# fluhus/frackyfrac

Hardware: NVIDIA B200
Metric: UniFrac sample-pairs/sec (unweighted) (higher is better)
Workload: dtype u8 x u8 -> s32 (tcgen05 kind::i8, exact), s64 chunk / row sums, f32 ratio / output

## Files before the change

frackyfrac_b200/csrc/embed.cu:

```cuda
#include "frc_internal.h"

namespace frc {

namespace {

constexpr int kThreads = 256;

__global__ void k_scatter_f64(const int64_t* __restrict__ row_ptr, const int32_t* __restrict__ col,
                              const double* __restrict__ val, int64_t s_base, int64_t s_end, double* E,
                              int64_t ld, int32_t* __restrict__ K, int32_t kp) {
  int64_t s = s_base + ((static_cast<int64_t>(blockIdx.x) * blockDim.x + threadIdx.x) >> 5);
  int lane = threadIdx.x & 31;
  if (s >= s_end) return;
  int64_t b = row_ptr[s], e = row_ptr[s + 1];
  for (int64_t k = b + lane; k < e; k += 32) {
    E[static_cast<int64_t>(col[k]) * ld + (s - s_base)] = val[k];
    if (K) K[((s >> 7) * kp + col[k]) * 128 + (s & 127)] = col[k];
  }
}

__global__ void k_level_sum_f64(const int32_t* __restrict__ nodes, const int32_t* __restrict__ child_ptr,
                                const int32_t* __restrict__ child_idx, double* E, int64_t ld,
                                int32_t* __restrict__ K, int32_t kp, int64_t s_base) {
  int32_t v = nodes[blockIdx.x];
  int64_t s = (static_cast<int64_t>(blockIdx.y) * blockDim.x + threadIdx.x) * 2;
  if (s >= ld) return;
  int32_t cb = child_ptr[v], ce = child_ptr[v + 1];
  double2 acc = make_double2(0.0, 0.0);
  for (int32_t c = cb; c < ce; ++c) {
    const double2 x = *reinterpret_cast<const double2*>(E + static_cast<int64_t>(child_idx[c]) * ld + s);
    acc.x = __dadd_rn(acc.x, x.x);
    acc.y = __dadd_rn(acc.y, x.y);
  }
  *reinterpret_cast<double2*>(E + static_cast<int64_t>(v) * ld + s) = acc;
  if (K) {
    const int64_t g = s_base + s;
    int32_t* const kt = K + (g >> 7) * kp * 128 + (g & 127);
    int2 key = make_int2(-1, -1);
    for (int32_t c = cb; c < ce; ++c) {
      const int2 x = *reinterpret_cast<const int2*>(kt + static_cast<int64_t>(child_idx[c]) * 128);
      key.x = max(key.x, x.x);
      key.y = max(key.y, x.y);
    }
    *reinterpret_cast<int2*>(kt + static_cast<int64_t>(v) * 128) = key;
  }
}

__global__ void k_totals_f64(const double* __restrict__ E, int32_t n_nodes, int64_t ld,
                             int64_t n_samples, double* __restrict__ total) {
  int64_t s = static_cast<int64_t>(blockIdx.x) * blockDim.x + threadIdx.x;
  if (s >= n_samples) return;
  double acc = 0.0;
  int32_t v = 0;
  for (; v + 8 <= n_nodes; v += 8) {
    double x[8];
#pragma unroll
    for (int u = 0; u < 8; ++u) x[u] = E[static_cast<int64_t>(v + u) * ld + s];
#pragma unroll
    for (int u = 0; u < 8; ++u) acc = __dadd_rn(acc, x[u]);
  }
  for (; v < n_nodes; ++v) acc = __dadd_rn(acc, E[static_cast<int64_t>(v) * ld + s]);
  total[s] = acc;
}

__global__ void k_normalize_f64(double* E, int32_t n_nodes, int64_t ld, int64_t n_samples,
                                const double* __restrict__ total) {
  int64_t s = static_cast<int64_t>(blockIdx.x) * blockDim.x + threadIdx.x;
  if (s >= n_samples) return;
  const double t = total[s];
  for (int32_t v = blockIdx.y; v < n_nodes; v += gridDim.y) {
    double x = E[static_cast<int64_t>(v) * ld + s];
    if (x != 0.0) E[static_cast<int64_t>(v) * ld + s] = __ddiv_rn(x, t);
  }
}

template <bool kMult>
__global__ void k_totals_partial_f64(const double* __restrict__ E, int32_t n_nodes, int64_t ld,
                                     const double* __restrict__ mult, double* __restrict__ partial) {
  int64_t s = static_cast<int64_t>(blockIdx.x) * blockDim.x + threadIdx.x;
  if (s >= ld) return;
  int32_t per = (n_nodes + gridDim.y - 1) / gridDim.y;
  int32_t v0 = blockIdx.y * per, v1 = min(n_nodes, v0 + per);
  auto term = [&](int32_t u) {
    const double x = E[static_cast<int64_t>(u) * ld + s];
    if constexpr (kMult) return mult[u] * x;
    else return x;
  };
  double a0 = 0.0, a1 = 0.0, a2 = 0.0, a3 = 0.0;
  int32_t v = v0;
  for (; v + 4 <= v1; v += 4) {
    a0 += term(v);
    a1 += term(v + 1);
    a2 += term(v + 2);
    a3 += term(v + 3);
  }
  for (; v < v1; ++v) a0 += term(v);
  partial[static_cast<int64_t>(blockIdx.y) * ld + s] = (a0 + a1) + (a2 + a3);
}

__global__ void k_weighted_operand(const double* __restrict__ E, const double* __restrict__ length,
                                   int32_t n_nodes, int64_t ld, const double* __restrict__ total,
                                   int prescale, float* __restrict__ A, double* __restrict__ partial) {
  int64_t s = static_cast<int64_t>(blockIdx.x) * blockDim.x + threadIdx.x;
  if (s >= ld) return;
  int32_t per = (n_nodes + gridDim.y - 1) / gridDim.y;
  int32_t v0 = blockIdx.y * per, v1 = min(n_nodes, v0 + per);
  const double t = total ? total[s] : 1.0;
  const double inv = t > 0.0 ? 1.0 / t : 0.0;
  double w = 0.0;
  for (int32_t v = v0; v < v1; ++v) {
    const double x = E[static_cast<int64_t>(v) * ld + s];
    const double a = total ? x * inv : x;
    const double la = length[v] * a;
    w += la;
    A[static_cast<int64_t>(v) * ld + s] = static_cast<float>(prescale ? la : a);
  }
  partial[static_cast<int64_t>(blockIdx.y) * ld + s] = w;
}

__global__ void k_weighted_operand_panels(const double* __restrict__ E, const double* __restrict__ length,
                                          int32_t n_nodes, int32_t kp, int64_t ld, int64_t s_base,
                                          const double* __restrict__ total, int prescale,
                                          float* __restrict__ Ap, double* __restrict__ partial) {
  int64_t ls = static_cast<int64_t>(blockIdx.x) * blockDim.x + threadIdx.x;
  if (ls >= ld) return;
  int32_t per = (n_nodes + gridDim.y - 1) / gridDim.y;
  int32_t v0 = blockIdx.y * per, v1 = min(n_nodes, v0 + per);
  const int64_t s = s_base + ls;
  float* dst = Ap + ((s >> 7) * kp) * 128 + (s & 127);
  const double t = total ? total[ls] : 1.0;
  const double inv = t > 0.0 ? 1.0 / t : 0.0;
  double w = 0.0;
  for (int32_t v = v0; v < v1; ++v) {
    const double x = E[static_cast<int64_t>(v) * ld + ls];
    const double a = total ? x * inv : x;
    const double la = length[v] * a;
    w += la;
    dst[static_cast<int64_t>(v) * 128] = static_cast<float>(prescale ? la : a);
  }
  if (blockIdx.y == gridDim.y - 1)
    for (int32_t v = n_nodes; v < kp; ++v) dst[static_cast<int64_t>(v) * 128] = 0.f;
  partial[static_cast<int64_t>(blockIdx.y) * ld + ls] = w;
}

__global__ void k_reduce_partials(const double* __restrict__ partial, int n_chunks, int64_t ld,
                                  int64_t n, double* __restrict__ out) {
  int64_t s = static_cast<int64_t>(blockIdx.x) * blockDim.x + threadIdx.x;
  if (s >= n) return;
  double acc = 0.0;
  for (int c = 0; c < n_chunks; ++c) acc += partial[static_cast<int64_t>(c) * ld + s];
  out[s] = acc;
}

// ... 142 lines not shown
#pragma unroll
    for (int u = 0; u < 8; ++u) {
      if (h + u < height) {
        if (n[u] >= 0) {
          const uint32_t x = colw[n[u]];
          if (x) atomicOr(colw + p[u], x);
        }
        __syncthreads();
      }
    }
  }
  uint32_t* dst = bitsT + static_cast<int64_t>(w) * kp;
  if (peers.n > 0) {
    const int64_t at = static_cast<int64_t>(w) * kp;
#pragma unroll 4
    for (int32_t k = tid; k < kp; k += 512) {
      const int32_t v = order[k];
      const uint32_t x = v >= 0 ? colw[v] : 0u;
#pragma unroll
      for (int pr = 0; pr < 8; ++pr)
        if (pr < peers.n) peers.p[pr][at + k] = x;
    }
  } else {
#pragma unroll 8
    for (int32_t k = tid; k < kp; k += 512) {
      const int32_t v = order[k];
      dst[k] = v >= 0 ? colw[v] : 0u;
    }
  }
  if (bitsS != nullptr) {
    const int32_t words = kp >> 5;
    for (int32_t g = warp; g * 128 < kp; g += 16) {
      uint32_t wout[4];
#pragma unroll
      for (int u = 0; u < 4; ++u) {
        const int32_t v = order[g * 128 + u * 32 + lane];
        const uint32_t wv = v >= 0 ? colw[v] : 0u;
        uint32_t mine = 0;
#pragma unroll
        for (int b = 0; b < 32; ++b) {
          const uint32_t bal = __ballot_sync(0xffffffffu, (wv >> b) & 1u);
          if (lane == b) mine = bal;
        }
        wout[u] = mine;
      }
      const int64_t srow = static_cast<int64_t>(w) * 32 + lane;
      *reinterpret_cast<uint4*>(bitsS + srow * words + g * 4) = make_uint4(wout[0], wout[1], wout[2], wout[3]);
    }
  }
}

__global__ void __launch_bounds__(32)
k_presence_rowsum_t(const uint32_t* __restrict__ bitsT, int32_t kp, int32_t per,
                    const double* __restrict__ lenq8, double* __restrict__ partial, int64_t ld, int32_t w0) {
  const int32_t w = blockIdx.x + w0, lane = threadIdx.x;
  const int32_t v0 = blockIdx.y * per, v1 = min(kp, v0 + per);
  const uint32_t* col = bitsT + static_cast<int64_t>(w) * kp;
  double a0 = 0.0, a1 = 0.0;
  for (int32_t v = v0; v < v1; v += 8) {
    const uint4 wa = *reinterpret_cast<const uint4*>(col + v), wb = *reinterpret_cast<const uint4*>(col + v + 4);
    const double2 l0 = *reinterpret_cast<const double2*>(lenq8 + v), l1 = *reinterpret_cast<const double2*>(lenq8 + v + 2);
    const double2 l2 = *reinterpret_cast<const double2*>(lenq8 + v + 4), l3 = *reinterpret_cast<const double2*>(lenq8 + v + 6);
    a0 += ((wa.x >> lane) & 1u) ? l0.x : 0.0;
    a1 += ((wa.y >> lane) & 1u) ? l0.y : 0.0;
    a0 += ((wa.z >> lane) & 1u) ? l1.x : 0.0;
    a1 += ((wa.w >> lane) & 1u) ? l1.y : 0.0;
    a0 += ((wb.x >> lane) & 1u) ? l2.x : 0.0;
    a1 += ((wb.y >> lane) & 1u) ? l2.y : 0.0;
    a0 += ((wb.z >> lane) & 1u) ? l3.x : 0.0;
    a1 += ((wb.w >> lane) & 1u) ? l3.y : 0.0;
  }
  partial[static_cast<int64_t>(blockIdx.y) * ld + w * 32 + lane] = a0 + a1;
}

__global__ void __launch_bounds__(32)
k_presence_rowsum_u8(const uint32_t* __restrict__ bitsT, int32_t kp, int32_t per,
                     const uint32_t* __restrict__ qam, const int32_t* __restrict__ col_exp,
                     double* __restrict__ partial, int64_t ld, int32_t w0, int32_t e_min,
                     long long* __restrict__ r_int) {
  const int32_t w = blockIdx.x + w0, lane = threadIdx.x;
  const int32_t v0 = blockIdx.y * per, v1 = min(kp, v0 + per);
  const uint32_t* col = bitsT + static_cast<int64_t>(w) * kp;
  const uint32_t m = 1u << lane;
  double tot = 0.0;
  unsigned long long tot_int = 0;
  for (int32_t blk = v0; blk < v1; blk += 128) {
    uint32_t a0 = 0, a1 = 0, a2 = 0, a3 = 0;
#pragma unroll 4
    for (int32_t v = blk; v < blk + 128; v += 8) {
      const uint4 wa = *reinterpret_cast<const uint4*>(col + v), wb = *reinterpret_cast<const uint4*>(col + v + 4);
      const uint4 qa = *reinterpret_cast<const uint4*>(qam + v), qb = *reinterpret_cast<const uint4*>(qam + v + 4);
      if (wa.x & m) a0 += qa.x;
      if (wa.y & m) a1 += qa.y;
      if (wa.z & m) a2 += qa.z;
      if (wa.w & m) a3 += qa.w;
      if (wb.x & m) a0 += qb.x;
      if (wb.y & m) a1 += qb.y;
      if (wb.z & m) a2 += qb.z;
      if (wb.w & m) a3 += qb.w;
    }
    const uint32_t sum = (a0 + a1) + (a2 + a3);
    const int32_t e = col_exp[blk];
    if (r_int) tot_int += static_cast<unsigned long long>(sum) << (e - e_min);
    else tot = fma(ldexp(1.0, e), static_cast<double>(sum), tot);
  }
  if (r_int) atomicAdd(reinterpret_cast<unsigned long long*>(r_int) + w * 32 + lane, tot_int);
  else partial[static_cast<int64_t>(blockIdx.y) * ld + w * 32 + lane] = tot;
}

__global__ void __launch_bounds__(256)
k_expand_operands_t(const uint32_t* __restrict__ bitsT, int32_t nw, int32_t kp,
                    int64_t np, const uint16_t* __restrict__ len_hi, const uint16_t* __restrict__ len_lo,
                    uint16_t* __restrict__ P, uint16_t* __restrict__ Bh, uint16_t* __restrict__ Bl,
                    const uint8_t* __restrict__ need) {
  __shared__ uint32_t words[8][64];
  const int32_t v0 = blockIdx.x * 64;
  const int32_t w0 = blockIdx.y * 8;
  const uint32_t nd = need ? need[blockIdx.y] : 3u;
  if (nd == 0u) return;
  for (int idx = threadIdx.x; idx < 512; idx += 256) {
    int word = idx >> 6, node = idx & 63;
    uint32_t x = 0;
    if (w0 + word < nw) x = bitsT[static_cast<int64_t>(w0 + word) * kp + v0 + node];
    words[word][node] = x;
  }
  __syncthreads();
  const int wi = threadIdx.x >> 5, lane = threadIdx.x & 31;
  const int32_t va = v0 + 2 * lane;
  const uint2 wab = *reinterpret_cast<const uint2*>(&words[wi][2 * lane]);
  const uint32_t wa = wab.x, wb = wab.y;
  const uint32_t hab = *reinterpret_cast<const uint32_t*>(len_hi + va);
  const uint32_t lab = *reinterpret_cast<const uint32_t*>(len_lo + va);
  const int64_t s0 = (static_cast<int64_t>(w0) + wi) * 32;
#pragma unroll 4
  for (int it = 0; it < 32; ++it) {
    const int64_t s = s0 + it;
    if (s >= np) break;
    const uint32_t m = (0xFFFFu & (0u - ((wa >> it) & 1u))) | (0xFFFF0000u & (0u - ((wb >> it) & 1u)));
    const int64_t o = s * kp + va;
    if (nd & 1u) *reinterpret_cast<uint32_t*>(P + o) = 0x3F803F80u & m;
    if (nd & 2u) {
      *reinterpret_cast<uint32_t*>(Bh + o) = hab & m;
      *reinterpret_cast<uint32_t*>(Bl + o) = lab & m;
    }
  }
}

__global__ void __launch_bounds__(256)
k_expand_operands_u8(const uint32_t* __restrict__ bitsT, int32_t nw, int32_t kp, int64_t np,
                     const uint8_t* __restrict__ qa, const uint8_t* __restrict__ qh,
                     const uint8_t* __restrict__ ql, uint8_t* __restrict__ A, uint8_t* __restrict__ Bh,
                     uint8_t* __restrict__ Bl, const uint8_t* __restrict__ need,
                     const uint32_t* __restrict__ qam, const int32_t* __restrict__ col_exp, int32_t e_min,
                     long long* __restrict__ r_int) {
  __shared__ __align__(16) uint32_t words[8][128];
  __shared__ __align__(16) uint32_t sq[128];
  const int32_t v0 = blockIdx.x * 128;
  const int32_t w0 = blockIdx.y * 8;
  const uint32_t nd = need ? need[blockIdx.y] : 3u;
  if (nd == 0u) return;
  for (int idx = threadIdx.x; idx < 1024; idx += 256) {
    int word = idx >> 7, node = idx & 127;
    uint32_t x = 0;
    if (w0 + word < nw) x = bitsT[static_cast<int64_t>(w0 + word) * kp + v0 + node];
    words[word][node] = x;
  }
  if (r_int != nullptr && threadIdx.x < 128) sq[threadIdx.x] = qam[v0 + threadIdx.x];
  __syncthreads();
  const int wi = threadIdx.x >> 5, lane = threadIdx.x & 31;
  const int32_t va = v0 + 4 * lane;
  const uint4 w4 = *reinterpret_cast<const uint4*>(&words[wi][4 * lane]);
  const uint32_t a4 = *reinterpret_cast<const uint32_t*>(qa + va);
  const uint32_t h4 = *reinterpret_cast<const uint32_t*>(qh + va);
  const uint32_t l4 = *reinterpret_cast<const uint32_t*>(ql + va);
  const int64_t s0 = (static_cast<int64_t>(w0) + wi) * 32;
#pragma unroll 4
  for (int it = 0; it < 32; ++it) {
    const int64_t s = s0 + it;
    if (s >= np) break;
    const uint32_t bits = ((w4.x >> it) & 1u) | (((w4.y >> it) & 1u) << 8) | (((w4.z >> it) & 1u) << 16) |
                          (((w4.w >> it) & 1u) << 24);
    const uint32_t m = bits * 0xFFu;
    const int64_t o = s * kp + va;
    if (nd & 1u) *reinterpret_cast<uint32_t*>(A + o) = a4 & m;
    if (nd & 2u) {
      *reinterpret_cast<uint32_t*>(Bh + o) = h4 & m;
      *reinterpret_cast<uint32_t*>(Bl + o) = l4 & m;
    }
  }
  if (r_int != nullptr) {
    const uint32_t m = 1u << lane;
    uint32_t a0 = 0, a1 = 0, a2 = 0, a3 = 0;
#pragma unroll 8
    for (int k = 0; k < 128; k += 4) {
      const uint4 w = *reinterpret_cast<const uint4*>(&words[wi][k]);
      const uint4 q = *reinterpret_cast<const uint4*>(&sq[k]);
      a0 += (w.x & m) ? q.x : 0u;
      a1 += (w.y & m) ? q.y : 0u;
      a2 += (w.z & m) ? q.z : 0u;
      a3 += (w.w & m) ? q.w : 0u;
    }
    const uint32_t sum = (a0 + a1) + (a2 + a3);
    const int64_t s = s0 + lane;
    if (sum != 0u && s < np)
      atomicAdd(reinterpret_cast<unsigned long long*>(r_int) + s,
                static_cast<unsigned long long>(sum) << (col_exp[v0] - e_min));
  }
}

__global__ void k_quantize_lengths(const double* __restrict__ len_col, const int32_t* __restrict__ col_exp,
                                   int32_t kp, uint8_t* __restrict__ qa, uint8_t* __restrict__ qh,
                                   uint8_t* __restrict__ ql, uint32_t* __restrict__ qam,
                                   double* __restrict__ lenq, double* __restrict__ qerr) {
  const int32_t k = blockIdx.x * blockDim.x + threadIdx.x;
  if (k >= kp) return;
  const double len = len_col[k];
  const int e = col_exp[k];
  const double x = ldexp(len, -e);
  int best_a = 0, best_m = 0;
  if (len > 0.0) {
    double best = 1e300;
    int a0 = static_cast<int>(ceil(x / 65535.0));
    if (a0 < 1) a0 = 1;
    for (int a = a0; a <= 255; ++a) {
      double m = rint(x / static_cast<double>(a));
      if (m > 65535.0) continue;
      if (m < 1.0) m = 1.0;
      const double err = fabs(static_cast<double>(a) * m - x);
      if (err < best) { best = err; best_a = a; best_m = static_cast<int>(m); }
    }
    if (best_a == 0) { best_a = 255; best_m = 65535; }
  }
  qa[k] = static_cast<uint8_t>(best_a);
  qh[k] = static_cast<uint8_t>(best_m >> 8);
  ql[k] = static_cast<uint8_t>(best_m & 255);
  qam[k] = static_cast<uint32_t>(best_a) * static_cast<uint32_t>(best_m);
  const double q = ldexp(static_cast<double>(best_a) * static_cast<double>(best_m), e);
  lenq[k] = q;
  const double err = fabs(q - len);
  qerr[k] = err > 2e-6 * len ? 1e6 * err : 0.0;
}

__global__ void __launch_bounds__(1024) k_sum_flag_u(const double* __restrict__ qerr, int32_t kp,
                                                     double* __restrict__ flag_u) {
  __shared__ double part[1024];
  double acc = 0.0;
  for (int32_t k = threadIdx.x; k < kp; k += 1024) acc += qerr[k];
  part[threadIdx.x] = acc;
  __syncthreads();
  for (int o = 512; o > 0; o >>= 1) {
    if (threadIdx.x < o) part[threadIdx.x] += part[threadIdx.x + o];
    __syncthreads();
  }
  if (threadIdx.x == 0) flag_u[0] = part[0];
}

}

int launch_embed_f64(const DevTree& t, const int32_t* level_ptr, const DevCsr& a, double* E,
                     int64_t ld, int64_t s_base, cudaStream_t s, int32_t* K, int32_t kp) {
  int launches = 0;
  cudaMemsetAsync(E, 0, sizeof(double) * ld * t.n_nodes, s);
  if (K) cudaMemsetAsync(K + (s_base >> 7) * kp * 128, 0xFF, sizeof(int32_t) * ld * kp, s);
  const int64_t s_end = s_base + ld < a.n_samples ? s_base + ld : a.n_samples;
  if (s_end > s_base && a.nnz > 0) {
    int64_t threads = (s_end - s_base) * 32;
    k_scatter_f64<<<static_cast<unsigned>((threads + kThreads - 1) / kThreads), kThreads, 0, s>>>(
        a.row_ptr, a.col, a.val, s_base, s_end, E, ld, K, kp);
    ++launches;
  }
  for (int32_t h = 1; h <= t.height; ++h) {
    int32_t b = level_ptr[h], e = level_ptr[h + 1];
    if (e == b) continue;
    dim3 grid(static_cast<unsigned>(e - b), static_cast<unsigned>((ld / 2 + kThreads - 1) / kThreads));
    k_level_sum_f64<<<grid, kThreads, 0, s>>>(t.level_nodes + b, t.child_ptr, t.child_idx, E, ld, K, kp, s_base);
    ++launches;
  }
  return launches;
}

static int pick_chunks(int32_t n_nodes) {
  int c = n_nodes / 256;
  return c < 1 ? 1 : (c > 64 ? 64 : c);
}

int launch_totals_fast_f64(const double* E, int32_t n_nodes, int64_t ld, const double* mult, double* total,
                           double* scratch, cudaStream_t s) {
  const int chunks = pick_chunks(n_nodes);
  dim3 grid(static_cast<unsigned>((ld + kThreads - 1) / kThreads), chunks);
  if (mult) k_totals_partial_f64<true><<<grid, kThreads, 0, s>>>(E, n_nodes, ld, mult, scratch);
  else k_totals_partial_f64<false><<<grid, kThreads, 0, s>>>(E, n_nodes, ld, nullptr, scratch);
  k_reduce_partials<<<static_cast<unsigned>((ld + kThreads - 1) / kThreads), kThreads, 0, s>>>(scratch, chunks, ld, ld,
                                                                                             total);
  return 2;
}

int launch_totals_f64(const double* E, int32_t n_nodes, int64_t ld, int64_t n_samples, double* total,
                      cudaStream_t s) {
  if (n_samples == 0) return 0;
  k_totals_f64<<<static_cast<unsigned>((n_samples + 127) / 128), 128, 0, s>>>(E, n_nodes, ld,
                                                                               n_samples, total);
  return 1;
}

int launch_normalize_f64(double* E, int32_t n_nodes, int64_t ld, int64_t n_samples,
                         const double* total, cudaStream_t s) {
  if (n_samples == 0) return 0;
  dim3 grid(static_cast<unsigned>((n_samples + kThreads - 1) / kThreads),
            static_cast<unsigned>(min(n_nodes, 512)));
  k_normalize_f64<<<grid, kThreads, 0, s>>>(E, n_nodes, ld, n_samples, total);
  return 1;
}


int launch_weighted_operand(const double* E, const double* length, int32_t n_nodes, int32_t kp,
                            int64_t ld, int64_t n_samples, const double* total, bool prescale,
                            float* A, double* W, double* scratch, cudaStream_t s) {
  int chunks = pick_chunks(n_nodes);
  if (kp > n_nodes)
    cudaMemsetAsync(A + static_cast<int64_t>(n_nodes) * ld, 0, sizeof(float) * ld * (kp - n_nodes), s);
  dim3 grid(static_cast<unsigned>((ld + kThreads - 1) / kThreads), chunks);
  k_weighted_operand<<<grid, kThreads, 0, s>>>(E, length, n_nodes, ld, total, prescale ? 1 : 0, A,
                                               scratch);
  k_reduce_partials<<<static_cast<unsigned>((ld + kThreads - 1) / kThreads), kThreads, 0, s>>>(
      scratch, chunks, ld, ld, W);
  (void)n_samples;
  return 2;
}
int launch_weighted_operand_panels(const double* E, const double* length, int32_t n_nodes, int32_t kp,
                                   int64_t ld, int64_t s_base, const double* total, bool prescale, float* Ap,
                                   double* W, double* scratch, cudaStream_t s) {
  int chunks = pick_chunks(n_nodes);
  dim3 grid(static_cast<unsigned>((ld + kThreads - 1) / kThreads), chunks);
  k_weighted_operand_panels<<<grid, kThreads, 0, s>>>(E, length, n_nodes, kp, ld, s_base, total, prescale ? 1 : 0,
                                                      Ap, scratch);
  k_reduce_partials<<<static_cast<unsigned>((ld + kThreads - 1) / kThreads), kThreads, 0, s>>>(
      scratch, chunks, ld, ld, W + s_base);
  return 2;
}
int weighted_scratch_chunks(int32_t n_nodes) { return pick_chunks(n_nodes); }

int launch_embed_bits(const DevTree& t, const int32_t* level_ptr, const DevCsr& a, uint32_t* bits,
                      int32_t nw, cudaStream_t s) {
  int launches = 0;
  cudaMemsetAsync(bits, 0, sizeof(uint32_t) * static_cast<int64_t>(nw) * t.n_nodes, s);
  if (a.n_samples > 0 && a.nnz > 0) {
    int64_t threads = a.n_samples * 32;
    k_scatter_bits<<<static_cast<unsigned>((threads + kThreads - 1) / kThreads), kThreads, 0, s>>>(
        a.row_ptr, a.col, a.n_samples, bits, nw);
    ++launches;
  }
  for (int32_t h = 1; h <= t.height; ++h) {
    int32_t b = level_ptr[h], e = level_ptr[h + 1];
    if (e == b) continue;
    dim3 grid(static_cast<unsigned>(e - b), static_cast<unsigned>((nw + 127) / 128));
    k_level_or<<<grid, 128, 0, s>>>(t.level_nodes + b, t.child_ptr, t.child_idx, bits, nw);
    ++launches;
  }
  return launches;
}

int launch_presence_rowsum(const uint32_t* bits, int32_t n_nodes, int32_t nw, const double* lenq,
                           double* r, double* scratch, cudaStream_t s) {
  int chunks = pick_chunks(n_nodes);
  dim3 grid(nw, chunks);
  k_presence_rowsum<<<grid, 32, 0, s>>>(bits, n_nodes, nw, lenq, scratch);
  int64_t ld = static_cast<int64_t>(nw) * 32;
  k_reduce_partials<<<static_cast<unsigned>((ld + kThreads - 1) / kThreads), kThreads, 0, s>>>(
      scratch, chunks, ld, ld, r);
  return 2;
}

int launch_expand_operands(const uint32_t* bits, int32_t n_nodes, int32_t nw, int32_t kp, int64_t np,
                           const uint16_t* len_hi, const uint16_t* len_lo, uint16_t* P, uint16_t* Bh,
                           uint16_t* Bl, cudaStream_t s) {
  dim3 grid(kp / 64, static_cast<unsigned>((np + 255) / 256));
  k_expand_operands<<<grid, 256, 0, s>>>(bits, n_nodes, nw, kp, np, len_hi, len_lo, P, Bh, Bl);
  return 1;
}


void embed_setup() {
  cudaFuncSetAttribute(k_embed_presence_fused<true>, cudaFuncAttributeMaxDynamicSharedMemorySize, 200 * 1024);
}

int64_t presence_node_scratch_words(int32_t n_nodes, int32_t nw) {
  return static_cast<size_t>(n_nodes) * 4 <= 200 * 1024 ? 0 : static_cast<int64_t>(n_nodes) * nw;
}

int launch_embed_presence_fused(const DevTree& t, const int32_t* level_ptr_dev, const DevCsr& a,
                                int32_t nw, int32_t w0, int32_t w_count, int32_t kp, const int32_t* order,
                                uint32_t* node_scratch, uint32_t* bitsT, uint32_t* bitsS, const PeerPtrs& peers,
                                cudaStream_t s) {
  (void)nw;
  const size_t smem = (static_cast<size_t>(t.n_nodes) * 4 + 15) & ~size_t(15);
  if (smem <= 200 * 1024) {
    k_embed_presence_fused<true><<<w_count, 512, smem, s>>>(a.row_ptr, a.col, a.n_samples, t.level_nodes,
                                                            t.level_parent, level_ptr_dev, t.height, t.n_nodes, kp,
                                                            order, node_scratch, bitsT, w0, bitsS, peers);
  } else {
    k_embed_presence_fused<false><<<w_count, 512, 0, s>>>(a.row_ptr, a.col, a.n_samples, t.level_nodes,
                                                          t.level_parent, level_ptr_dev, t.height, t.n_nodes, kp,
                                                          order, node_scratch, bitsT, w0, bitsS, peers);
  }
  return 1;
}

int launch_presence_rowsum_t(const uint32_t* bitsT, int32_t n_nodes, int32_t nw, int32_t w0, int32_t w_count,
                             int32_t kp, const double* lenq, const uint32_t* qam, const int32_t* col_exp,
                             double* partial, double* r, int32_t e_min, long long* r_int, cudaStream_t s) {
  const int64_t np = static_cast<int64_t>(nw) * 32;
  const int chunks = pick_chunks(n_nodes);
  dim3 g(w_count, chunks);
  const int64_t s0 = static_cast<int64_t>(w0) * 32, ns = static_cast<int64_t>(w_count) * 32;
  if (qam) {
    const int32_t per = static_cast<int32_t>(round_up((kp + chunks - 1) / chunks, 128));
    if (r_int) cudaMemsetAsync(r_int + s0, 0, sizeof(long long) * ns, s);
    k_presence_rowsum_u8<<<g, 32, 0, s>>>(bitsT, kp, per, qam, col_exp, partial, np, w0, e_min, r_int);
    if (r_int) return 1;
  } else {
    const int32_t per = static_cast<int32_t>(round_up((kp + chunks - 1) / chunks, 8));
    k_presence_rowsum_t<<<g, 32, 0, s>>>(bitsT, kp, per, lenq, partial, np, w0);
  }
  k_reduce_partials<<<static_cast<unsigned>((ns + kThreads - 1) / kThreads), kThreads, 0, s>>>(partial + s0, chunks, np,
                                                                                              ns, r + s0);
  return 2;
}

int launch_expand_operands_t(const uint32_t* bitsT, int32_t nw, int32_t kp, int64_t np, bool i8,
                             const void* q0, const void* q1, const void* q2, void* P, void* Bh, void* Bl,
                             const uint8_t* need, const uint32_t* qam, const int32_t* col_exp, int32_t e_min,
                             long long* r_int, cudaStream_t s) {
  if (i8) {
    if (r_int) cudaMemsetAsync(r_int, 0, sizeof(long long) * np, s);
    dim3 grid(kp / 128, static_cast<unsigned>((np + 255) / 256));
    k_expand_operands_u8<<<grid, 256, 0, s>>>(bitsT, nw, kp, np, static_cast<const uint8_t*>(q0),
                                              static_cast<const uint8_t*>(q1), static_cast<const uint8_t*>(q2),
                                              static_cast<uint8_t*>(P), static_cast<uint8_t*>(Bh),
                                              static_cast<uint8_t*>(Bl), need, qam, col_exp, e_min, r_int);
  } else {
    (void)q0;
    dim3 grid(kp / 64, static_cast<unsigned>((np + 255) / 256));
    k_expand_operands_t<<<grid, 256, 0, s>>>(bitsT, nw, kp, np, static_cast<const uint16_t*>(q1),
                                             static_cast<const uint16_t*>(q2), static_cast<uint16_t*>(P),
                                             static_cast<uint16_t*>(Bh), static_cast<uint16_t*>(Bl), need);
  }
  return 1;
}

int launch_quantize_lengths(const double* len_col, const int32_t* col_exp, int32_t kp, uint8_t* qa,
                            uint8_t* qh, uint8_t* ql, uint32_t* qam, double* lenq, double* qerr, double* flag_u,
                            cudaStream_t s) {
  k_quantize_lengths<<<(kp + 127) / 128, 128, 0, s>>>(len_col, col_exp, kp, qa, qh, ql, qam, lenq, qerr);
  k_sum_flag_u<<<1, 1024, 0, s>>>(qerr, kp, flag_u);
  return 2;
}

}
```

frackyfrac_b200/csrc/frc_internal.h:

```cpp
#pragma once
#include <cuda_runtime.h>
#include <cstdint>
#include <string>

namespace frc {

constexpr int kTile = 128;
constexpr int kKBlock = 64;

inline int64_t round_up(int64_t x, int64_t m) { return (x + m - 1) / m * m; }
inline int64_t tri(int64_t i) { return i * (i - 1) / 2; }

struct DevTree {
  int32_t n_nodes = 0;
  int32_t height = 0;
  const int32_t* parent = nullptr;
  const double* length = nullptr;
  const int32_t* child_ptr = nullptr;
  const int32_t* child_idx = nullptr;
  const int32_t* level_nodes = nullptr;
  const int32_t* level_parent = nullptr;
};

struct DevCsr {
  int64_t n_samples = 0;
  int64_t nnz = 0;
  const int64_t* row_ptr = nullptr;
  const int32_t* col = nullptr;
  const double* val = nullptr;
};

struct PeerPtrs {
  uint32_t* p[8] = {nullptr, nullptr, nullptr, nullptr, nullptr, nullptr, nullptr, nullptr};
  int n = 0;
  int self = 0;
};

struct Tile { int32_t ti, tj; };

struct Exceptions {
  unsigned long long* count = nullptr;
  int64_t* index = nullptr;
  double* value = nullptr;
  int32_t cap = 0;
};

int launch_embed_f64(const DevTree& t, const int32_t* level_ptr_host, const DevCsr& a, double* E,
                     int64_t ld, int64_t s_base, cudaStream_t s, int32_t* K = nullptr, int32_t kp = 0);
int launch_totals_f64(const double* E, int32_t n_nodes, int64_t ld, int64_t n_samples,
                      double* total, cudaStream_t s);
int launch_totals_fast_f64(const double* E, int32_t n_nodes, int64_t ld, const double* mult, double* total,
                           double* scratch, cudaStream_t s);
int launch_normalize_f64(double* E, int32_t n_nodes, int64_t ld, int64_t n_samples,
                         const double* total, cudaStream_t s);
int launch_weighted_operand(const double* E, const double* length, int32_t n_nodes, int32_t kp,
                            int64_t ld, int64_t n_samples, const double* total, bool prescale,
                            float* A, double* W, double* scratch, cudaStream_t s);
int launch_weighted_operand_panels(const double* E, const double* length, int32_t n_nodes, int32_t kp,
                                   int64_t ld, int64_t s_base, const double* total, bool prescale, float* Ap,
                                   double* W, double* scratch, cudaStream_t s);
int weighted_scratch_chunks(int32_t n_nodes);

int launch_embed_bits(const DevTree& t, const int32_t* level_ptr_host, const DevCsr& a,
                      uint32_t* bits, int32_t nw, cudaStream_t s);
int launch_presence_rowsum(const uint32_t* bits, int32_t n_nodes, int32_t nw, const double* lenq,
                           double* r, double* scratch, cudaStream_t s);
int launch_expand_operands(const uint32_t* bits, int32_t n_nodes, int32_t nw, int32_t kp,
                           int64_t np, const uint16_t* len_hi, const uint16_t* len_lo,
                           uint16_t* P, uint16_t* Bh, uint16_t* Bl, cudaStream_t s);

int64_t presence_node_scratch_words(int32_t n_nodes, int32_t nw);
void embed_setup();
int launch_embed_presence_fused(const DevTree& t, const int32_t* level_ptr_dev, const DevCsr& a,
                                int32_t nw, int32_t w0, int32_t w_count, int32_t kp, const int32_t* order,
                                uint32_t* node_scratch, uint32_t* bitsT, uint32_t* bitsS, const PeerPtrs& peers,
                                cudaStream_t s);
int launch_presence_rowsum_t(const uint32_t* bitsT, int32_t n_nodes, int32_t nw, int32_t w0, int32_t w_count,
                             int32_t kp, const double* lenq, const uint32_t* qam, const int32_t* col_exp,
                             double* partial, double* r, int32_t e_min, long long* r_int, cudaStream_t s);
int launch_expand_operands_t(const uint32_t* bitsT, int32_t nw, int32_t kp, int64_t np, bool i8,
                             const void* q0, const void* q1, const void* q2, void* P, void* Bh, void* Bl,
                             const uint8_t* need, const uint32_t* qam, const int32_t* col_exp, int32_t e_min,
                             long long* r_int, cudaStream_t s);
int launch_quantize_lengths(const double* len_col, const int32_t* col_exp, int32_t kp, uint8_t* qa,
                            uint8_t* qh, uint8_t* ql, uint32_t* qam, double* lenq, double* qerr, double* flag_u,
                            cudaStream_t s);

struct Comm;
bool comm_unique_id(char* id128, std::string* err);
Comm* comm_create(const char* id128, int rank, int world, std::string* err);
void comm_destroy(Comm* c);
int comm_rank(const Comm* c);
int comm_world(const Comm* c);
bool comm_all_gather_inplace(Comm* c, void* const* bufs, const size_t* bytes_per_rank, int n, cudaStream_t s,
                             std::string* err);

bool comm_all_gather_host(Comm* c, const void* mine, size_t bytes, void* all, cudaStream_t s, std::string* err);
bool comm_barrier(Comm* c, cudaStream_t s, std::string* err);

int launch_exact_pairs(const double* E, const double* length, int32_t n_nodes, int64_t ld,
                       bool weighted, int64_t first, int64_t count, double* out, cudaStream_t s);
int launch_postorder_lists(const double* E, const int32_t* post_order, int32_t n_nodes, int64_t ld, int64_t n_samples,
                           int64_t* list_ptr, int32_t* list_id, double* list_val, cudaStream_t s);
int launch_unsorted_pairs(const int64_t* list_ptr, const int32_t* list_id, const double* list_val,
                          const double* length, int64_t first, int64_t count, double* out, cudaStream_t s);

void widen_band(const float* src, double* dst, int64_t n, bool stream_stores);

struct PanelMap {
  const float* shard[16] = {nullptr, nullptr, nullptr, nullptr, nullptr, nullptr, nullptr, nullptr,
                            nullptr, nullptr, nullptr, nullptr, nullptr, nullptr, nullptr, nullptr};
  int32_t n_shards = 0;
  int32_t tiles_per_shard = 0;
};
int launch_weighted_tiles(const PanelMap& A, int64_t ld, int32_t kp, const float* lenf, bool prescaled,
                          const double* W, const Tile* tiles, int32_t n_tiles, int64_t n_samples,
                          int64_t first, float* out, double flag_below, uint32_t* flagged,
                          unsigned long long* n_flagged, int num_sms, cudaStream_t s, const int32_t* K = nullptr);
int launch_weighted_fixup(const DevCsr& a, const DevTree& t, const double* total, const double* W,
                          const uint32_t* flagged, const unsigned long long* n_flagged,
                          unsigned long long* count_host, int64_t first, long long* ws, int ws_ctas, float* out,
                          const Exceptions& ex, cudaStream_t s, const int32_t* K = nullptr, int32_t kp = 0);
void weighted_setup();

struct TcOperands;
struct TcChunks {
  const int32_t* end = nullptr;
  const double* scale = nullptr;
  const int32_t* shift = nullptr;
  int32_t n = 0;
  bool biased = false;
};
TcOperands* tc_operands_create(const void* P, const void* Bh, const void* Bl, int64_t np, int32_t kp,
                               bool i8, const TcChunks& chunks, const double* len_col, const double* flag_u,
                               std::string* err);
TcOperands* tc_operands_create_bits(const uint32_t* bitsS, int64_t np, int32_t kp, const uint8_t* qa,
                                    const uint8_t* qh, const uint8_t* ql, const TcChunks& chunks,
                                    const double* len_col, const double* flag_u, const long long* r_int,
                                    double unit, std::string* err);
void tc_operands_set_int(TcOperands* o, const long long* r_int, double unit);
void tc_operands_destroy(TcOperands* o);
int tc_chunk_kblocks();
int launch_unweighted_tc(const TcOperands* ops, const double* r, const Tile* tiles, int32_t n_tiles,
                         int64_t n_samples, int64_t first, float* out, double flag_below,
                         uint32_t* flagged, unsigned long long* n_flagged, int num_sms, cudaStream_t s);
int launch_unweighted_fixup(const TcOperands* ops, const uint32_t* flagged,
                            const unsigned long long* n_flagged, unsigned long long* count_host,
                            int64_t first, float* out, const Exceptions& ex, int num_sms, cudaStream_t s);
bool tc_setup(std::string* err);

}
```

frackyfrac_b200/csrc/job.cu:

```cuda
#include <algorithm>
#include <atomic>
#include <chrono>
#include <climits>
#include <cmath>
#include <cstdio>
#include <cstdlib>
#include <cstring>
#include <functional>
#include <memory>
#include <string>
#include <thread>
#include <vector>

#if defined(__x86_64__)
#include <immintrin.h>
#endif

#include "../../include/frcfrc_cuda.h"
#include "frc_internal.h"
#include "host_pool.h"
#include "plan.h"

using namespace frc;
using frc_host::Pool;
// ... 66 lines not shown
  int ws_slab = 0;
  bool uw_bf16 = false;
  bool u8_acc_f64 = false;
  bool feed_bits = false;
  bool embed_levels = false;
  int peer_push = -1;
  int group_binades = 3;
  int shard = -1;
  int capacity = -1;
  static Knobs read() {
    Knobs k;
    auto num = [](const char* name, int dflt) { const char* e = getenv(name); return e && *e ? atoi(e) : dflt; };
    auto is = [](const char* name, const char* v) { const char* e = getenv(name); return e && !strcmp(e, v); };
    k.trace = getenv("FRC_TRACE") != nullptr;
    k.bands_per_rank = std::max(0, num("FRC_BANDS", 0));
    k.widen_threads = std::max(0, num("FRC_WIDEN_THREADS", 0));
    k.ws_slab = std::max(0, num("FRC_WS_SLAB", 0));
    k.uw_bf16 = is("FRC_UW_KERNEL", "bf16");
    k.u8_acc_f64 = is("FRC_U8_ACC", "f64");
    k.feed_bits = is("FRC_UW_FEED", "bits");
    k.embed_levels = num("FRC_EMBED_LEVELS", 0) == 1;
    k.peer_push = num("FRC_PEER_PUSH", -1);
    k.group_binades = num("FRC_U8_GROUP_BINADES", 3);
    k.shard = num("FRC_SHARD", -1);
    k.capacity = num("FRC_CAPACITY", -1);
    return k;
  }
};

struct DeviceGuard {
  int prev = -1;
  DeviceGuard() { if (cudaGetDevice(&prev) != cudaSuccess) { prev = -1; cudaGetLastError(); } }
  ~DeviceGuard() { if (prev >= 0) cudaSetDevice(prev); }
};

}

struct DevCtx {
  int device = 0;
  int num_sms = 0;
  cudaStream_t stream[4] = {nullptr, nullptr, nullptr, nullptr};
  Arena dev, pin, sym;
};

struct frc_ctx {
  std::vector<DevCtx*> devs;
  Arena pin;
  std::unique_ptr<Pool> pool;
  std::vector<std::vector<int64_t>> stamps;
  int64_t stamp_epoch = 0;
  bool in_use = false;
  bool peer_ok = false;
  Comm* comm = nullptr;
  std::vector<std::vector<char*>> sym_peer;
};

namespace {

struct Slot {
  double* dev64 = nullptr;
  double* host64 = nullptr;
  float* dev32 = nullptr;
  float* host32 = nullptr;
  uint32_t* flagged = nullptr;
  unsigned long long* n_flagged_host = nullptr;
  Exceptions ex;
  cudaEvent_t k0 = nullptr, k1 = nullptr, k2 = nullptr, done = nullptr;
  int band = -1;
};

struct Seg { size_t off = 0, bytes = 0; };
struct SegAlloc {
  size_t total = 0;
  Seg operator()(size_t bytes) { Seg s{total, bytes}; total += (bytes + 255) & ~size_t(255); return s; }
};

struct Shared {
  frc_opts_t opts{};
  Knobs knobs;
  int64_t N = 0, np = 0, nnz = 0;
  int32_t B = 0, kp = 0, nw = 0;
  bool exact = false, weighted = false, prescale = true, need_val = false;
  bool unsorted_l = false;
  bool keyed = false;
  bool node_mult = false;
  bool d2h = true;
  int n_parts = 1;
  int world = 1, rank0 = 0;
  enum Exchange { kNone, kInProcess, kNccl } exchange = kNone;
  bool fused_embed = true, bits_feed = false;
  bool capacity = false;
  ShardPlan shards;
  ColumnPlan cols;
  std::vector<Band> bands;
  std::vector<int32_t> level_ptr;
  int32_t tree_height = 0;
  char* stage_in = nullptr;
  Seg in_rowptr, in_parent, in_len, in_cptr, in_cidx, in_lvl, in_lpar, in_lptr, in_lenf, in_post, in_mult, in_col, in_val;
  size_t in_bytes = 0;
  char* stage_plan = nullptr;
  Seg pl_q0, pl_hi, pl_lo, pl_lenq, pl_order, pl_cexp, pl_lcol, pl_cend, pl_cscale, pl_cshift;
  size_t plan_bytes = 0;
};

}

struct frc_job;

namespace {

struct Part {
  frc_job* job = nullptr;
  const Shared* sh = nullptr;
  DevCtx* dc = nullptr;
  int index = 0;
  int owner = 0;
  int rc = FRC_OK;
  std::string err;
  frc_info_t info{};

  std::vector<int> mine;
  std::vector<Band> bands;
  std::vector<Tile> tiles;

  int32_t shard_w0 = 0, shard_nw = 0;
  int64_t csr_k0 = 0, csr_k1 = 0;
  PanelMap pm;
  struct CapGroup {
    int shard = 0;
    int64_t first = 0, count = 0;
    int32_t tile_off = 0;
    std::vector<int32_t> coff;
    float* out = nullptr;
    uint32_t* flagged = nullptr;
    unsigned long long* cnt = nullptr;
    unsigned long long* n_flagged_host = nullptr;
    Exceptions ex;
    cudaEvent_t done = nullptr;
    bool counted = false;
  };
  std::vector<CapGroup> cap;
  std::vector<int> band_group;
  float* d_V[2] = {nullptr, nullptr};
  std::vector<cudaEvent_t> ev_fetch, ev_used;

  DevTree dtree;
  DevCsr dcsr;
  char* d_in = nullptr;
  char* d_plan = nullptr;
  Tile* d_tiles = nullptr;
  int32_t* d_level_ptr = nullptr;
  int32_t* d_post = nullptr;
  unsigned long long* d_flag_counts = nullptr;
  int64_t ws_slab = 0;
  bool peer_push = false;
  uint32_t* d_bits2[2] = {nullptr, nullptr};
  PeerPtrs peers[2];
  int64_t run_count = 0;
  void *d_q0 = nullptr, *d_q1 = nullptr, *d_q2 = nullptr;
  int32_t *d_order = nullptr, *d_col_exp = nullptr;
  uint32_t* d_qam = nullptr;
  uint32_t* d_bitsS = nullptr;
  long long* d_r_int = nullptr;
  long long* d_fix_ws[2] = {nullptr, nullptr};
  uint8_t* d_need = nullptr;
  double *d_lenq = nullptr, *d_len_col = nullptr, *d_flag_u = nullptr, *d_qerr = nullptr;
  TcChunks d_chunks;
  float* d_lenf = nullptr;
  const double* d_mult = nullptr;
  double *d_E = nullptr, *d_total = nullptr, *d_W = nullptr, *d_r = nullptr, *d_scratch = nullptr;
  float* d_A = nullptr;
  int32_t* d_K = nullptr;
  uint32_t *d_bits = nullptr, *d_node_scratch = nullptr;
  void *d_P = nullptr, *d_Bh = nullptr, *d_Bl = nullptr;
  TcOperands* tc = nullptr;
  int64_t* d_list_ptr = nullptr;
  int32_t* d_list_id = nullptr;
  double* d_list_val = nullptr;
  int64_t list_cap = 0;

  Slot slots[kSlots];
  int n_slots = 0;
  int64_t max_band = 1;
  size_t next_enqueue = 0, next_deliver = 0;
  cudaEvent_t ev_h2d0 = nullptr, ev_h2d1 = nullptr, ev_embed0 = nullptr, ev_embed1 = nullptr;
  cudaEvent_t ev_run1 = nullptr, ev_join = nullptr, ev_bits = nullptr, ev_rsum = nullptr;
  cudaEvent_t ev_shard = nullptr;
  bool run_timed = false, embed_timed = false;
  std::chrono::steady_clock::time_point t_host0;
};

}

struct frc_job {
  frc_ctx* ctx = nullptr;
  bool own_ctx = false;
  Shared sh;
  std::vector<std::unique_ptr<Part>> parts;
  std::string err;
  frc_info_t info{};
  struct Item { int part, idx; };
  std::vector<Item> order;
  size_t next_item = 0;
  int held_part = -1;
  int held_slot = -1;
  int64_t held_first = 0, held_count = 0;
  std::vector<int64_t> ex_index;
  std::vector<double> ex_value;
  int read_mode = 0;
  double* wide = nullptr;
  int64_t piece_first = 0, piece_off = 0, piece_end = 0;
  double create_ms = 0;
};

namespace {

#define PART_CUDA(p, expr)                                                                   \
  do {                                                                                       \
    cudaError_t _e = (expr);                                                                 \
    if (_e != cudaSuccess) {                                                                 \
      (p)->err = std::string(#expr) + ": " + cudaGetErrorString(_e);                         \
      cudaGetLastError();                                                                    \
      return (p)->rc = (_e == cudaErrorMemoryAllocation ? FRC_ERR_OOM : FRC_ERR_CUDA);       \
    }                                                                                        \
  } while (0)

int pfail(Part* p, int code, const std::string& msg) { p->err = msg; return p->rc = code; }
int fail(frc_job* j, int code, const std::string& msg) { j->err = msg; return code; }

template <class T>
T* dev_alloc(Part* p, size_t n) {
  cudaError_t e = cudaSuccess;
  void* q = p->dc->dev.alloc(n * sizeof(T), &e);
  if (!q) {
    p->err = "device allocation of " + std::to_string(n * sizeof(T)) + " bytes failed: " + cudaGetErrorString(e);
    p->rc = FRC_ERR_OOM;
  }
  return static_cast<T*>(q);
}
template <class T>
T* pin_alloc(Part* p, size_t n) {
  cudaError_t e = cudaSuccess;
  void* q = p->dc->pin.alloc(n * sizeof(T), &e);
  if (!q) {
    p->err = "pinned host allocation of " + std::to_string(n * sizeof(T)) + " bytes failed: " + cudaGetErrorString(e);
    p->rc = FRC_ERR_OOM;
  }
  return static_cast<T*>(q);
}

int for_parts(frc_job* j, const std::function<int(Part*)>& fn) {
  const int n = static_cast<int>(j->parts.size());
  if (n == 1) {
    cudaSetDevice(j->parts[0]->dc->device);
    fn(j->parts[0].get());
  } else {
    Pool* pool = j->ctx->pool.get();
    const int T = std::min(n, pool->size());
    std::atomic<int> next{0};
    pool->run(T, [&](int) {
      for (int k = next.fetch_add(1); k < n; k = next.fetch_add(1)) {
        cudaSetDevice(j->parts[k]->dc->device);
        fn(j->parts[k].get());
      }
    });
  }
  for (auto& p : j->parts)
    if (p->rc) { j->err = p->err; return p->rc; }
  return FRC_OK;
}

int sym_sync(Part* p, bool* usable) {
  frc_ctx* c = p->job->ctx;
  DevCtx* dc = p->dc;
  const int world = comm_world(c->comm), rank = comm_rank(c->comm);
  char failed = 0;
  while (c->sym_peer.size() < dc->sym.blocks.size()) {
    const size_t b = c->sym_peer.size();
    cudaIpcMemHandle_t mine;
    memset(&mine, 0, sizeof(mine));
    if (cudaIpcGetMemHandle(&mine, dc->sym.blocks[b].p) != cudaSuccess) { cudaGetLastError(); failed = 1; }
    std::vector<cudaIpcMemHandle_t> all(world);
    std::string cerr;
    if (!comm_all_gather_host(c->comm, &mine, sizeof(mine), all.data(), dc->stream[0], &cerr))
      return pfail(p, FRC_ERR_CUDA, cerr);
    std::vector<char*> bases(world, nullptr);
    for (int r = 0; r < world; ++r) {
      if (r == rank) { bases[r] = dc->sym.blocks[b].p; continue; }
      void* q = nullptr;
      if (failed || cudaIpcOpenMemHandle(&q, all[r], cudaIpcMemLazyEnablePeerAccess) != cudaSuccess) {
        cudaGetLastError();
        failed = 1;
        q = nullptr;
      }
      bases[r] = static_cast<char*>(q);
    }
    c->sym_peer.push_back(bases);
  }
  for (auto& blk : c->sym_peer)
    for (char* base : blk)
      if (!base) failed = 1;
  std::vector<char> flags(world, 0);
  std::string cerr;
  if (!comm_all_gather_host(c->comm, &failed, 1, flags.data(), dc->stream[0], &cerr)) return pfail(p, FRC_ERR_CUDA, cerr);
  *usable = true;
  for (char f : flags) if (f) *usable = false;
  return FRC_OK;
}

struct ShardArray {
  void* (*on)(const Part*);
  size_t sample_bytes;
  bool copy = true;
};
template <auto M> void* part_array(const Part* q) { return q->*M; }

int exchange_shard(Part* p, const std::vector<ShardArray>& arrs, const Range& rg, cudaStream_t s) {
  const Shared& sh = *p->sh;
  if (sh.exchange == Shared::kNone) return FRC_OK;
  const size_t n = static_cast<size_t>(rg.s1 - rg.s0);
  const int others = (sh.exchange == Shared::kNccl ? sh.world : sh.n_parts) - 1;
  std::vector<void*> bufs;
  std::vector<size_t> bytes;
  for (const ShardArray& a : arrs) {
    p->info.gather_bytes += static_cast<int64_t>(n * a.sample_bytes) * others;
    if (a.copy) { bufs.push_back(a.on(p)); bytes.push_back(n * a.sample_bytes); }
  }
  if (sh.exchange == Shared::kNccl) {
    Comm* comm = p->job->ctx->comm;
    std::string cerr;
    const bool ok = bufs.empty() ? comm_barrier(comm, s, &cerr)
                                 : comm_all_gather_inplace(comm, bufs.data(), bytes.data(), static_cast<int>(bufs.size()), s, &cerr);
    return ok ? FRC_OK : pfail(p, FRC_ERR_CUDA, cerr);
  }
  for (int q = 0; q < sh.n_parts; ++q) {
    if (q == p->index) continue;
    const Part* o = p->job->parts[q].get();
    for (const ShardArray& a : arrs) {
      if (!a.copy) continue;
      const size_t off = rg.s0 * a.sample_bytes;
      PART_CUDA(p, cudaMemcpyPeerAsync(static_cast<char*>(a.on(o)) + off, o->dc->device, static_cast<char*>(a.on(p)) + off,
                                       p->dc->device, n * a.sample_bytes, s));
    }
  }
  return FRC_OK;
}

int embed_stage1(Part* p) {
  const Shared& sh = *p->sh;
  DevCtx* dc = p->dc;
  frc_ctx* c = p->job->ctx;
  cudaStream_t s = dc->stream[0];
  int launches = 0;
  p->t_host0 = std::chrono::steady_clock::now();
  if (p->d_flag_counts)
    PART_CUDA(p, cudaMemsetAsync(p->d_flag_counts, 0, sizeof(unsigned long long) * (p->mine.size() + 1), s));
  PART_CUDA(p, cudaEventRecord(p->ev_embed0, s));
  p->info.gather_bytes = 0;
  const bool inproc = sh.exchange == Shared::kInProcess;
  if (sh.exact) {
    launches += launch_embed_f64(p->dtree, sh.level_ptr.data(), p->dcsr, p->d_E, sh.np, 0, s);
    if (sh.opts.normalize == 1 && sh.weighted) {
      launches += launch_totals_f64(p->d_E, sh.B, sh.np, sh.N, p->d_total, s);
      launches += launch_normalize_f64(p->d_E, sh.B, sh.np, sh.N, p->d_total, s);
    }
    if (sh.unsorted_l) {
      launches += launch_postorder_lists(p->d_E, p->d_post, sh.B, sh.np, sh.N, p->d_list_ptr, nullptr, nullptr, s);
      int64_t total = 0;
      PART_CUDA(p, cudaMemcpyAsync(&total, p->d_list_ptr + sh.N, sizeof(int64_t), cudaMemcpyDeviceToHost, s));
      PART_CUDA(p, cudaStreamSynchronize(s));
      if (total > p->list_cap) {
        p->list_cap = total;
        if (!(p->d_list_id = dev_alloc<int32_t>(p, static_cast<size_t>(total) + 1))) return p->rc;
        if (!(p->d_list_val = dev_alloc<double>(p, static_cast<size_t>(total) + 1))) return p->rc;
      }
      launches += launch_postorder_lists(p->d_E, p->d_post, sh.B, sh.np, sh.N, p->d_list_ptr, p->d_list_id,
                                         p->d_list_val, s);
    }
    p->info.embed_bytes = 2LL * sh.B * sh.np * 8 + 12LL * sh.nnz;
  } else if (sh.weighted) {
    const bool norm = sh.opts.normalize == 1;
    std::vector<ShardArray> arrs;
    if (!sh.capacity) arrs.push_back({part_array<&Part::d_A>, sizeof(float) * sh.kp});
    arrs.push_back({part_array<&Part::d_W>, sizeof(double)});
    if (norm) arrs.push_back({part_array<&Part::d_total>, sizeof(double)});
    if (sh.keyed) arrs.push_back({part_array<&Part::d_K>, sizeof(int32_t) * sh.kp});
    int64_t built = 0;
    for (const Range& rg : sh.shards.ranges[p->owner]) {
      built += rg.s1 - rg.s0;
      const int64_t shift = (rg.slot * sh.shards.shard_rows - rg.s0) * sh.kp;
      float* Ap = p->d_A + shift;
      int32_t* Kp = sh.keyed ? p->d_K + shift : nullptr;
      for (int64_t sb = rg.s0; sb < rg.s1; sb += p->ws_slab) {
        const int64_t ld = std::min<int64_t>(p->ws_slab, rg.s1 - sb);
        launches += launch_embed_f64(p->dtree, sh.level_ptr.data(), p->dcsr, p->d_E, ld, sb, s, Kp, sh.kp);
        if (norm) launches += launch_totals_fast_f64(p->d_E, sh.B, ld, p->d_mult, p->d_total + sb, p->d_scratch, s);
        launches += launch_weighted_operand_panels(p->d_E, p->dtree.length, sh.B, sh.kp, ld, sb,
                                                   norm ? p->d_total + sb : nullptr, sh.prescale, Ap, p->d_W,
                                                   p->d_scratch, s);
      }
      if (exchange_shard(p, arrs, rg, s)) return p->rc;
    }
    p->pm = PanelMap{};
    if (sh.capacity) {
      p->pm.n_shards = sh.shards.n_shards;
      p->pm.tiles_per_shard = static_cast<int32_t>(sh.shards.shard_rows / kTile);
      for (int k = 0; k < sh.shards.n_shards; ++k)
        if (sh.shards.owner[k] == p->owner) p->pm.shard[k] = p->d_A + sh.shards.slot[k] * sh.shards.shard_rows * sh.kp;
    } else {
      p->pm.shard[0] = p->d_A;
    }
    p->info.embed_bytes = 2LL * sh.B * built * (sh.keyed ? 12 : 8) + 12LL * (p->csr_k1 - p->csr_k0);
  } else if (sh.fused_embed) {
    const int cur = static_cast<int>(p->run_count & 1);
    if (p->peer_push) {
      p->d_bits = p->d_bits2[cur];
      if (p->run_count == 0) {
        std::string cerr;
        if (!comm_barrier(c->comm, s, &cerr)) return pfail(p, FRC_ERR_CUDA, cerr);
      }
    }
    ++p->run_count;
    PeerPtrs peers;
    if (p->peer_push) peers = p->peers[cur];
    else if (inproc && !sh.bits_feed) {
      peers.n = sh.n_parts; peers.self = p->index;
      for (int q = 0; q < sh.n_parts; ++q) peers.p[q] = p->job->parts[q]->d_bits;
    }
    launches += launch_embed_presence_fused(p->dtree, p->d_level_ptr, p->dcsr, sh.nw, p->shard_w0, p->shard_nw,
                                            sh.kp, p->d_order, p->d_node_scratch, p->d_bits, p->d_bitsS, peers, s);
    const bool rowsum_in_expand = sh.cols.intacc && !sh.bits_feed;
    const bool split = sh.exchange == Shared::kNone && !rowsum_in_expand;
    cudaStream_t rs = split ? dc->stream[1] : s;
    if (split) {
      PART_CUDA(p, cudaEventRecord(p->ev_bits, s));
      PART_CUDA(p, cudaStreamWaitEvent(rs, p->ev_bits, 0));
    }
    if (!rowsum_in_expand)
      launches += launch_presence_rowsum_t(p->d_bits, sh.B, sh.nw, p->shard_w0, p->shard_nw, sh.kp, p->d_lenq,
                                           sh.cols.i8 ? p->d_qam : nullptr, p->d_col_exp, p->d_scratch, p->d_r,
                                           sh.cols.e_min, sh.cols.intacc ? p->d_r_int : nullptr, rs);
    std::vector<ShardArray> arrs;
    if (!rowsum_in_expand)
      arrs.push_back({sh.cols.intacc ? part_array<&Part::d_r_int> : part_array<&Part::d_r>, sizeof(double)});
    arrs.push_back({sh.bits_feed ? part_array<&Part::d_bitsS> : part_array<&Part::d_bits>, sizeof(uint32_t) * sh.kp / 32,
                    peers.n == 0});
    if (exchange_shard(p, arrs, sh.shards.ranges[p->owner][0], s)) return p->rc;
    if (sh.exchange != Shared::kNone) {
      p->info.embed_bytes = 2LL * sh.B * p->shard_nw * 4 + 4LL * (p->csr_k1 - p->csr_k0);
    }
  }
  PART_CUDA(p, cudaGetLastError());
  if (inproc) PART_CUDA(p, cudaEventRecord(p->ev_shard, s));
  p->info.kernel_launches += launches;
  return FRC_OK;
}

int embed_stage2(Part* p) {
  const Shared& sh = *p->sh;
  DevCtx* dc = p->dc;
  cudaStream_t s = dc->stream[0];
  int launches = 0;
  if (sh.exchange == Shared::kInProcess)
    for (auto& o : p->job->parts)
      if (o.get() != p) PART_CUDA(p, cudaStreamWaitEvent(s, o->ev_shard, 0));
  if (!sh.exact && !sh.weighted) {
    if (sh.fused_embed) {
      const bool rowsum_in_expand = sh.cols.intacc && !sh.bits_feed;
      if (!sh.bits_feed)
        launches += launch_expand_operands_t(p->d_bits, sh.nw, sh.kp, sh.np, sh.cols.i8, p->d_q0, p->d_q1, p->d_q2,
                                             p->d_P, p->d_Bh, p->d_Bl, p->d_need, p->d_qam, p->d_col_exp, sh.cols.e_min,
                                             rowsum_in_expand ? p->d_r_int : nullptr, s);
      if (sh.exchange == Shared::kNone) {
        if (!rowsum_in_expand) {
          PART_CUDA(p, cudaEventRecord(p->ev_rsum, dc->stream[1]));
          PART_CUDA(p, cudaStreamWaitEvent(s, p->ev_rsum, 0));
        }
        p->info.embed_bytes = 2LL * sh.B * sh.nw * 4 + 4LL * sh.nnz;
      }
      if (!sh.bits_feed) p->info.embed_bytes += 3LL * sh.np * sh.kp * (sh.cols.i8 ? 1 : 2) + 4LL * sh.nw * sh.kp;
    } else {
      launches += launch_embed_bits(p->dtree, sh.level_ptr.data(), p->dcsr, p->d_bits, sh.nw, s);
      launches += launch_presence_rowsum(p->d_bits, sh.B, sh.nw, p->d_lenq, p->d_r, p->d_scratch, s);
      launches += launch_expand_operands(p->d_bits, sh.B, sh.nw, sh.kp, sh.np,
                                         static_cast<const uint16_t*>(p->d_q1), static_cast<const uint16_t*>(p->d_q2),
                                         static_cast<uint16_t*>(p->d_P), static_cast<uint16_t*>(p->d_Bh),
                                         static_cast<uint16_t*>(p->d_Bl), s);
      p->info.embed_bytes = 2LL * sh.B * sh.nw * 4 + 3LL * sh.np * sh.kp * 2 + 4LL * sh.nnz;
    }
  }
  PART_CUDA(p, cudaGetLastError());
  PART_CUDA(p, cudaEventRecord(p->ev_embed1, s));
  PART_CUDA(p, cudaStreamWaitEvent(dc->stream[1], p->ev_embed1, 0));
  p->info.kernel_launches += launches;
  p->embed_timed = false;
  return FRC_OK;
}

int enqueue_band(Part* p, size_t idx) {
  const Shared& sh = *p->sh;
  DevCtx* dc = p->dc;
  if (sh.knobs.trace)
    fprintf(stderr, "[host] dev %d enqueue band %zu at %.3f ms\n", dc->device, idx,
            std::chrono::duration<double, std::milli>(std::chrono::steady_clock::now() - p->t_host0).count());
  const Band& b = p->bands[idx];
  Slot& sl = p->slots[idx % p->n_slots];
  const int si = static_cast<int>(idx % 2);
  cudaStream_t s = dc->stream[si];
  sl.band = static_cast<int>(idx);
  int launches = 0;
  if (sh.capacity) {
    Part::CapGroup& cb = p->cap[p->band_group[idx]];
    cudaStream_t cs = dc->stream[2];
    float* band_out = cb.out + (b.first - cb.first);
    sl.dev32 = band_out; sl.flagged = cb.flagged; sl.ex = cb.ex;
    sl.n_flagged_host = cb.counted ? nullptr : cb.n_flagged_host;
    cb.counted = true;
    PART_CUDA(p, cudaStreamWaitEvent(cs, cb.done, 0));
    for (cudaEvent_t e : {sl.k0, sl.k1, sl.k2}) PART_CUDA(p, cudaEventRecord(e, cs));
    if (sh.d2h) {
      PART_CUDA(p, cudaMemcpyAsync(sl.host32, band_out, sizeof(float) * b.count, cudaMemcpyDeviceToHost, cs));
      p->info.d2h_bytes += static_cast<int64_t>(sizeof(float)) * b.count;
    }
    PART_CUDA(p, cudaEventRecord(sl.done, cs));
    if (idx + 1 == p->mine.size()) {
      PART_CUDA(p, cudaStreamWaitEvent(dc->stream[0], sl.done, 0));
      PART_CUDA(p, cudaEventRecord(p->ev_run1, dc->stream[0]));
    }
    return FRC_OK;
  }
  PART_CUDA(p, cudaEventRecord(sl.k0, s));
  if (sh.exact) {
    if (sh.unsorted_l)
      launches += launch_unsorted_pairs(p->d_list_ptr, p->d_list_id, p->d_list_val, p->dtree.length, b.first, b.count,
                                        sl.dev64, s);
    else
      launches += launch_exact_pairs(p->d_E, p->dtree.length, sh.B, sh.np, sh.weighted, b.first, b.count, sl.dev64, s);
    PART_CUDA(p, cudaEventRecord(sl.k1, s));
  } else {
    unsigned long long* cnt = p->d_flag_counts + idx;
    *sl.ex.count = 0;
    if (sh.weighted) {
      launches += launch_weighted_tiles(p->pm, sh.np, sh.kp, p->d_lenf, sh.prescale, p->d_W, p->d_tiles + b.tile_off,
                                        b.n_tiles, sh.N, b.first, sl.dev32, kFlagBelowW, sl.flagged, cnt, dc->num_sms, s,
                                        p->d_K);
      PART_CUDA(p, cudaEventRecord(sl.k1, s));
      launches += launch_weighted_fixup(p->dcsr, p->dtree, sh.opts.normalize == 1 ? p->d_total : nullptr, p->d_W,
                                        sl.flagged, cnt, sl.n_flagged_host, b.first, p->d_fix_ws[si], kFixupCtas,
                                        sl.dev32, sl.ex, s, p->d_K, sh.kp);
    } else {
      launches += launch_unweighted_tc(p->tc, p->d_r, p->d_tiles + b.tile_off, b.n_tiles, sh.N, b.first, sl.dev32,
                                       kFlagBelow, sl.flagged, cnt, dc->num_sms, s);
      PART_CUDA(p, cudaEventRecord(sl.k1, s));
      launches += launch_unweighted_fixup(p->tc, sl.flagged, cnt, sl.n_flagged_host, b.first, sl.dev32, sl.ex,
                                          dc->num_sms, s);
    }
  }
  PART_CUDA(p, cudaGetLastError());
  PART_CUDA(p, cudaEventRecord(sl.k2, s));
  if (sh.d2h) {
    cudaStream_t cs = dc->stream[2];
    PART_CUDA(p, cudaStreamWaitEvent(cs, sl.k2, 0));
    if (sh.exact) {
      PART_CUDA(p, cudaMemcpyAsync(sl.host64, sl.dev64, sizeof(double) * b.count, cudaMemcpyDeviceToHost, cs));
      p->info.d2h_bytes += static_cast<int64_t>(sizeof(double)) * b.count;
    } else {
      PART_CUDA(p, cudaMemcpyAsync(sl.host32, sl.dev32, sizeof(float) * b.count, cudaMemcpyDeviceToHost, cs));
      p->info.d2h_bytes += static_cast<int64_t>(sizeof(float)) * b.count;
    }
    PART_CUDA(p, cudaEventRecord(sl.done, cs));
  } else {
    PART_CUDA(p, cudaEventRecord(sl.done, s));
  }
  p->info.kernel_launches += launches;
  if (idx + 1 == p->mine.size()) {
    PART_CUDA(p, cudaEventRecord(p->ev_join, dc->stream[1]));
    PART_CUDA(p, cudaStreamWaitEvent(dc->stream[0], p->ev_join, 0));
    PART_CUDA(p, cudaStreamWaitEvent(dc->stream[0], sl.done, 0));
    PART_CUDA(p, cudaEventRecord(p->ev_run1, dc->stream[0]));
  }
  return FRC_OK;
}

int start_pairs_capacity(Part* p) {
  const Shared& sh = *p->sh;
  DevCtx* dc = p->dc;
  cudaStream_t s = dc->stream[0], cin = dc->stream[3];
  const ShardPlan& sp = sh.shards;
  const size_t shard_floats = static_cast<size_t>(sp.shard_rows) * sh.kp;
  int launches = 0, n_remote = 0, last_c = 0;
  for (const Part::CapGroup& cb : p->cap) last_c = std::max(last_c, cb.shard);
  PanelMap pm = p->pm;
  int prev_user[2] = {-1, -1};
  int64_t fetched = 0;
  for (Part::CapGroup& cb : p->cap) { *cb.ex.count = 0; cb.counted = false; }
  PART_CUDA(p, cudaMemsetAsync(p->cap[0].cnt, 0, sizeof(unsigned long long) * p->cap.size(), s));
  for (int c = 0; c <= last_c; ++c) {
    const bool remote = sp.owner[c] != p->index;
    if (remote) {
      const int buf = n_remote++ & 1;
      Part* o = p->job->parts[sp.owner[c]].get();
      const float* src = o->d_A + sp.slot[c] * shard_floats;
      if (prev_user[buf] >= 0) PART_CUDA(p, cudaStreamWaitEvent(cin, p->ev_used[prev_user[buf]], 0));
      PART_CUDA(p, cudaStreamWaitEvent(cin, o->ev_shard, 0));
      PART_CUDA(p, cudaMemcpyPeerAsync(p->d_V[buf], dc->device, src, o->dc->device, shard_floats * sizeof(float), cin));
      PART_CUDA(p, cudaEventRecord(p->ev_fetch[c], cin));
      PART_CUDA(p, cudaStreamWaitEvent(s, p->ev_fetch[c], 0));
      pm.shard[c] = p->d_V[buf];
      prev_user[buf] = c;
      fetched += static_cast<int64_t>(shard_floats * sizeof(float));
    }
    for (Part::CapGroup& cb : p->cap) {
      if (cb.shard < c) continue;
      const int32_t t0 = cb.coff[c], n = cb.coff[c + 1] - cb.coff[c];
      launches += launch_weighted_tiles(pm, sh.np, sh.kp, p->d_lenf, sh.prescale, p->d_W, p->d_tiles + cb.tile_off + t0, n,
                                        sh.N, cb.first, cb.out, kFlagBelowW, cb.flagged, cb.cnt, dc->num_sms, s);
      if (cb.shard == c) {
        launches += launch_weighted_fixup(p->dcsr, p->dtree, sh.opts.normalize == 1 ? p->d_total : nullptr, p->d_W,
                                          cb.flagged, cb.cnt, cb.n_flagged_host, cb.first, p->d_fix_ws[0], kFixupCtas,
                                          cb.out, cb.ex, s);
        PART_CUDA(p, cudaEventRecord(cb.done, s));
      }
    }
    PART_CUDA(p, cudaGetLastError());
    if (remote) PART_CUDA(p, cudaEventRecord(p->ev_used[c], s));
  }
  p->info.gather_bytes += fetched;
  p->info.kernel_launches += launches;
  return FRC_OK;
}

int start_pairs(Part* p) {
  p->next_enqueue = p->next_deliver = 0;
  p->info.pairs_ms = 0;
  p->info.fixup_ms = 0;
  p->info.run_ms = 0;
  p->run_timed = false;
  p->info.flagged_pairs = 0;
  p->info.exceptions = 0;
  p->info.d2h_bytes = 0;
  if (p->mine.empty()) {
    PART_CUDA(p, cudaEventRecord(p->ev_run1, p->dc->stream[0]));
    return FRC_OK;
  }
  if (p->sh->capacity && start_pairs_capacity(p)) return p->rc;
  while (p->next_enqueue < p->mine.size() && p->next_enqueue < static_cast<size_t>(p->n_slots - 1)) {
    if (enqueue_band(p, p->next_enqueue)) return p->rc;
    ++p->next_enqueue;
  }
  return FRC_OK;
}

void destroy_part(Part* p) {
  if (!p) return;
  if (p->dc) {
    cudaSetDevice(p->dc->device);
    for (auto s : p->dc->stream) if (s) cudaStreamSynchronize(s);
    cudaGetLastError();
  }
  for (auto& sl : p->slots) {
    if (sl.k0) cudaEventDestroy(sl.k0);
    if (sl.k1) cudaEventDestroy(sl.k1);
    if (sl.k2) cudaEventDestroy(sl.k2);
    if (sl.done) cudaEventDestroy(sl.done);
  }
  for (cudaEvent_t e : {p->ev_h2d0, p->ev_h2d1, p->ev_embed0, p->ev_embed1, p->ev_run1, p->ev_join, p->ev_bits,
                        p->ev_rsum, p->ev_shard})
    if (e) cudaEventDestroy(e);
  for (cudaEvent_t e : p->ev_fetch) if (e) cudaEventDestroy(e);
  for (cudaEvent_t e : p->ev_used) if (e) cudaEventDestroy(e);
  for (auto& cb : p->cap) if (cb.done) cudaEventDestroy(cb.done);
  tc_operands_destroy(p->tc);
  if (p->dc) {
    p->dc->dev.reset();
    p->dc->pin.reset();
    p->dc->sym.reset();
  }
}

void destroy_job(frc_job* j) {
  if (!j) return;
  for (auto& p : j->parts)
    if (p->dc) {
      cudaSetDevice(p->dc->device);
      for (auto s : p->dc->stream) if (s) cudaStreamSynchronize(s);
    }
  cudaGetLastError();
  for (auto& p : j->parts) destroy_part(p.get());
  if (j->ctx) {
    j->ctx->pin.reset();
    j->ctx->in_use = false;
    if (j->own_ctx) frc_ctx_destroy(j->ctx);
  }
  delete j;
}

int make_dev_ctx(int device, DevCtx** out) {
  cudaError_t e;
  cudaDeviceProp prop;
  if ((e = cudaGetDeviceProperties(&prop, device)) != cudaSuccess) {
    g_create_error = std::string("cudaGetDeviceProperties: ") + cudaGetErrorString(e);
    return FRC_ERR_CUDA;
  }
  if (prop.major != 10) {
    g_create_error = "libfrcfrc_cuda is built for sm_100a (B200) only; device " + std::to_string(device) +
                     " is sm_" + std::to_string(prop.major) + std::to_string(prop.minor) + " (" + prop.name + ")";
    return FRC_ERR_UNSUPPORTED;
  }
  if ((e = cudaSetDevice(device)) != cudaSuccess) {
    g_create_error = std::string("cudaSetDevice: ") + cudaGetErrorString(e);
    return FRC_ERR_CUDA;
  }
  DevCtx* d = new DevCtx();
  d->device = device;
  d->num_sms = prop.multiProcessorCount;
  d->dev.pinned = false; d->dev.min_block = 64u << 20;
  d->sym.pinned = false; d->sym.min_block = 32u << 20;
  d->pin.pinned = true;  d->pin.min_block = 8u << 20;
  *out = d;
  for (auto& s : d->stream)
    if ((e = cudaStreamCreateWithFlags(&s, cudaStreamNonBlocking)) != cudaSuccess) {
      g_create_error = std::string("cudaStreamCreate: ") + cudaGetErrorString(e);
      return FRC_ERR_CUDA;
    }
  std::string terr;
  if (!tc_setup(&terr)) { g_create_error = terr; return FRC_ERR_CUDA; }
  weighted_setup();
  embed_setup();
  if ((e = cudaGetLastError()) != cudaSuccess) {
    g_create_error = std::string("kernel attribute setup: ") + cudaGetErrorString(e);
    return FRC_ERR_CUDA;
  }
  return FRC_OK;
}

}

extern "C" {

int frc_abi_version(void) { return FRC_ABI_VERSION; }

const char* frc_last_error(const frc_job_t* job) { return job ? job->err.c_str() : g_create_error.c_str(); }

int frc_ctx_create_multi(int32_t n_devices, const int32_t* devices, frc_ctx_t** out) {
  if (!out) { g_create_error = "frc_ctx_create: out is NULL"; return FRC_ERR_ARG; }
  *out = nullptr;
  int count = 0;
  cudaError_t e = cudaGetDeviceCount(&count);
  if (e != cudaSuccess || count == 0) {
    cudaGetLastError();
    g_create_error = std::string("no CUDA device: ") + (e != cudaSuccess ? cudaGetErrorString(e) : "count is 0");
    return FRC_ERR_CUDA;
  }
  DeviceGuard guard;
  std::vector<int> ids;
  if (n_devices < 0) {
    for (int d = 0; d < count && static_cast<int>(ids.size()) < kMaxParts; ++d) {
      cudaDeviceProp prop;
      if (cudaGetDeviceProperties(&prop, d) == cudaSuccess && prop.major == 10) ids.push_back(d);
    }
    if (ids.empty()) { g_create_error = "no sm_100 device visible (libfrcfrc_cuda is built for B200 only)"; return FRC_ERR_UNSUPPORTED; }
  } else {
    if (n_devices == 0) n_devices = 1;
    if (n_devices > kMaxParts) { g_create_error = "at most 8 devices per job"; return FRC_ERR_UNSUPPORTED; }
    for (int k = 0; k < n_devices; ++k) {
      int d = devices ? devices[k] : k;
      if (n_devices == 1 && d < 0) { if (guard.prev >= 0) d = guard.prev; else d = 0; }
      if (d < 0 || d >= count) { g_create_error = "device ordinal out of range"; return FRC_ERR_ARG; }
      for (int x : ids) if (x == d) { g_create_error = "device listed twice"; return FRC_ERR_ARG; }
      ids.push_back(d);
    }
  }
  frc_ctx* c = new frc_ctx();
  c->pin.pinned = true; c->pin.min_block = 8u << 20;
  for (int d : ids) {
    DevCtx* dc = nullptr;
    int rc = make_dev_ctx(d, &dc);
    if (dc) c->devs.push_back(dc);
    if (rc) { frc_ctx_destroy(c); return rc; }
  }
  if (c->devs.size() > 1) {
    bool ok = true;
    for (DevCtx* a : c->devs)
      for (DevCtx* b : c->devs) {
        if (a == b) continue;
        int can = 0;
        if (cudaDeviceCanAccessPeer(&can, a->device, b->device) != cudaSuccess || !can) { ok = false; continue; }
        cudaSetDevice(a->device);
        cudaError_t pe = cudaDeviceEnablePeerAccess(b->device, 0);
        if (pe != cudaSuccess && pe != cudaErrorPeerAccessAlreadyEnabled) ok = false;
        cudaGetLastError();
      }
    c->peer_ok = ok;
  }
  {
    int hw = static_cast<int>(std::thread::hardware_concurrency());
    int n = std::max(1, std::min(16, hw));
    if (c->devs.size() > 1) n = std::max(n, std::min(hw, 32));
    if (const char* ev = getenv("FRC_HOST_THREADS")) n = std::max(1, atoi(ev));
    c->pool.reset(new Pool(n - 1));
    c->stamps.resize(n);
  }
  *out = c;
  return FRC_OK;
}

int frc_ctx_create(int32_t device, frc_ctx_t** out) { return frc_ctx_create_multi(1, &device, out); }

void frc_ctx_destroy(frc_ctx_t* c) {
  if (!c) return;
  DeviceGuard guard;
  c->pool.reset();
  for (DevCtx* d : c->devs) {
    cudaSetDevice(d->device);
    for (auto s : d->stream) if (s) cudaStreamSynchronize(s);
  }
  if (!c->devs.empty()) {
    DevCtx* d0 = c->devs[0];
    cudaSetDevice(d0->device);
    for (size_t b = 0; b < c->sym_peer.size(); ++b)
// ... 105 lines not shown
  sh.in_mult = seg(sh.node_mult ? sizeof(double) * B : 0);
  sh.in_col = seg(sizeof(int32_t) * sh.nnz);
  sh.in_val = seg(sh.need_val ? sizeof(double) * sh.nnz : 0);
  sh.in_bytes = seg.total;
}

int plan_job(frc_job* j, const frc_tree_t* tree, bool neg_len) {
  Shared& sh = j->sh;
  frc_ctx* c = j->ctx;
  const int n_parts = sh.n_parts;
  const bool fast_uw = !sh.exact && !sh.weighted;
  sh.fused_embed = !sh.knobs.embed_levels;
  sh.exchange = Shared::kNone;
  if (!sh.exact) {
    if (n_parts > 1 && c->peer_ok && sh.knobs.shard != 0 && (sh.weighted || sh.fused_embed)) sh.exchange = Shared::kInProcess;
    if (n_parts == 1 && sh.world > 1 && (sh.opts.flags & FRC_FLAG_SHARD_EMBED)) {
      if (!c->comm || comm_world(c->comm) != sh.world || comm_rank(c->comm) != sh.rank0)
        return fail(j, FRC_ERR_STATE, "FRC_FLAG_SHARD_EMBED needs a context whose communicator "
                                      "(frc_ctx_comm_init) matches opts->rank / opts->world");
      if (fast_uw && !sh.fused_embed) return fail(j, FRC_ERR_UNSUPPORTED, "FRC_EMBED_LEVELS=1 cannot build a sample shard");
      sh.exchange = Shared::kNccl;
    }
  }
  const int owners = sh.n_parts > 1 ? sh.n_parts : sh.world;
  ShardPlan::Mode mode = sh.exchange == Shared::kNone ? ShardPlan::kWhole : ShardPlan::kSharded;
  if (sh.exchange == Shared::kInProcess && sh.weighted && sh.knobs.capacity != 0 && sh.N >= 2) {
    bool want = sh.knobs.capacity == 1;
    if (!want) {
      const double panels = (sh.keyed ? 8.0 : 4.0) * static_cast<double>(round_up(sh.B, kKBlock)) * static_cast<double>(plan_shards(sh.N, n_parts, ShardPlan::kCapacity).np);
      if (panels > 24.0 * (1 << 30)) {
        size_t free_b = 0, total_b = 0;
        cudaSetDevice(c->devs[0]->device);
        if (cudaMemGetInfo(&free_b, &total_b) == cudaSuccess && panels > 0.55 * static_cast<double>(free_b)) want = true;
        cudaGetLastError();
      }
    }
    if (want && sh.keyed)
      return fail(j, FRC_ERR_UNSUPPORTED, "the key-matched tiles of -l as coded (FRC_FLAG_L_TILES) keep the value and key "
                                          "panels of all samples on every device; the capacity mode, which shards them "
                                          "over the devices when they exceed about half of one device's free HBM (or with "
                                          "FRC_CAPACITY=1), does not carry keys");
    sh.capacity = want;
    if (want) mode = ShardPlan::kCapacity;
  }
  sh.shards = plan_shards(sh.N, owners, mode);
  sh.np = sh.shards.np;
  sh.nw = static_cast<int32_t>(sh.np / 32);
  sh.kp = static_cast<int32_t>(round_up(sh.B, kKBlock));
  sh.prescale = !neg_len;
  if (fast_uw) {
    const bool want_i8 = sh.fused_embed && !neg_len && !(sh.opts.flags & FRC_FLAG_UW_BF16) && !sh.knobs.uw_bf16;
    sh.cols = plan_columns(tree->length, sh.B, want_i8, sh.knobs.group_binades, sh.knobs.u8_acc_f64, tc_chunk_kblocks());
    sh.kp = sh.cols.kp;
    sh.bits_feed = sh.cols.intacc && ((sh.opts.flags & FRC_FLAG_UW_BITS) != 0 || sh.knobs.feed_bits);
    if (sh.cols.intacc && !sh.bits_feed) {
      const double need = 3.0 * static_cast<double>(sh.np) * sh.kp;
      if (need > 32.0 * (1 << 30)) {
        size_t free_b = 0, total_b = 0;
        cudaSetDevice(c->devs[0]->device);
        if (cudaMemGetInfo(&free_b, &total_b) == cudaSuccess && need > 0.80 * static_cast<double>(free_b)) sh.bits_feed = true;
        cudaGetLastError();
      }
    }
  }
  sh.bands = sh.capacity ? make_bands_capacity(sh.N, sh.shards, sh.opts.band_rows, sh.d2h)
                         : make_bands(sh.N, sh.opts.band_rows, owners, sh.d2h, sh.knobs.bands_per_rank, 8);
  for (const Band& b : sh.bands)
    if (b.count >= (1LL << 32)) return fail(j, FRC_ERR_UNSUPPORTED, "band too large; lower band_rows");
  return FRC_OK;
}

int stage_plan(frc_job* j, const frc_tree_t* tree) {
  Shared& sh = j->sh;
  const ColumnPlan& cp = sh.cols;
  SegAlloc seg;
  sh.pl_q0 = seg(sh.kp); sh.pl_hi = seg(sizeof(uint16_t) * sh.kp); sh.pl_lo = seg(sizeof(uint16_t) * sh.kp);
  sh.pl_lenq = seg(sizeof(double) * sh.kp);
  sh.pl_order = seg(sizeof(int32_t) * cp.col_order.size()); sh.pl_cexp = seg(sizeof(int32_t) * cp.col_exp.size());
  sh.pl_lcol = seg(sizeof(double) * cp.len_col.size()); sh.pl_cend = seg(sizeof(int32_t) * cp.chunk_end.size());
  sh.pl_cscale = seg(sizeof(double) * cp.chunk_scale.size()); sh.pl_cshift = seg(sizeof(int32_t) * cp.chunk_shift.size());
  sh.plan_bytes = seg.total;
  cudaError_t e = cudaSuccess;
  sh.stage_plan = static_cast<char*>(j->ctx->pin.alloc(sh.plan_bytes, &e));
  if (!sh.stage_plan) return fail(j, FRC_ERR_OOM, std::string("pinned staging: ") + cudaGetErrorString(e));
  char* st = sh.stage_plan;
  if (!sh.exact && !sh.weighted && !cp.i8) {
    uint16_t* hi = reinterpret_cast<uint16_t*>(st + sh.pl_hi.off);
    uint16_t* lo = reinterpret_cast<uint16_t*>(st + sh.pl_lo.off);
    double* lq = reinterpret_cast<double*>(st + sh.pl_lenq.off);
    for (int32_t v = 0; v < sh.B; ++v) {
      const double l = tree->length[v];
      hi[v] = bf16_rn(static_cast<float>(l));
      const double res = l - static_cast<double>(bf16_to_float(hi[v]));
      lo[v] = (l == l && !std::isinf(l)) ? bf16_rn(static_cast<float>(res)) : 0;
      lq[v] = static_cast<double>(bf16_to_float(hi[v])) + static_cast<double>(bf16_to_float(lo[v]));
    }
    for (int32_t v = sh.B; v < sh.kp; ++v) { hi[v] = 0; lo[v] = 0; lq[v] = 0.0; }
  }
  auto put = [&](const Seg& s, const void* src) { if (s.bytes) memcpy(st + s.off, src, s.bytes); };
  put(sh.pl_order, cp.col_order.data()); put(sh.pl_cexp, cp.col_exp.data()); put(sh.pl_lcol, cp.len_col.data());
  put(sh.pl_cend, cp.chunk_end.data()); put(sh.pl_cscale, cp.chunk_scale.data()); put(sh.pl_cshift, cp.chunk_shift.data());
  return FRC_OK;
}

int prepare_part(Part* p) {
  const Shared& sh = *p->sh;
  DevCtx* dc = p->dc;
  frc_ctx* c = p->job->ctx;
  const int32_t B = sh.B;
  PART_CUDA(p, cudaSetDevice(dc->device));
  p->max_band = 1;
  for (size_t k = 0; k < sh.bands.size(); ++k)
    if (sh.bands[k].owner == p->owner) {
      p->mine.push_back(static_cast<int>(k));
      p->bands.push_back(sh.bands[k]);
      p->info.n_pairs_mine += sh.bands[k].count;
      p->max_band = std::max(p->max_band, sh.bands[k].count);
    }
  const bool fast_uw = !sh.exact && !sh.weighted;
  if (sh.capacity) {
    const std::vector<CapGroupPlan> groups =
        plan_capacity_groups(p->bands, sh.N, sh.shards.shard_rows, sh.shards.n_shards, p->tiles, p->band_group);
    for (const CapGroupPlan& gp : groups) {
      if (gp.count >= (1LL << 32)) return pfail(p, FRC_ERR_UNSUPPORTED, "capacity mode: a row shard holds 2^32 pairs or more");
      Part::CapGroup g;
      g.shard = gp.shard; g.first = gp.first; g.count = gp.count; g.tile_off = gp.tile_off; g.coff = gp.coff;
      p->cap.push_back(g);
    }
  } else if (!sh.exact) {
    for (Band& b : p->bands) append_band_tiles(b, fast_uw, p->tiles);
  }
  std::vector<uint8_t> need;
  if (fast_uw && sh.shards.ranges.size() > 1 && sh.fused_embed) need = operand_need_blocks(p->tiles, sh.np, true);
  const Range& own = sh.shards.ranges[p->owner][0];
  p->shard_w0 = static_cast<int32_t>(own.s0 / 32);
  p->shard_nw = static_cast<int32_t>((own.s1 - own.s0) / 32);
  p->csr_k0 = 0; p->csr_k1 = sh.nnz;
  if (sh.exchange != Shared::kNone && fast_uw && sh.N > 0) {
    const int64_t* rp = reinterpret_cast<const int64_t*>(sh.stage_in + sh.in_rowptr.off);
    p->csr_k0 = rp[std::min(sh.N, own.s0)]; p->csr_k1 = rp[std::min(sh.N, own.s1)];
  }
  SegAlloc seg;
  const Seg s_tiles = seg(sizeof(Tile) * p->tiles.size()), s_need = seg(need.size());
  char* st = pin_alloc<char>(p, seg.total);
  if (!st) return p->rc;
  char* d_small = dev_alloc<char>(p, seg.total);
  if (!d_small) return p->rc;
  if (!p->tiles.empty()) memcpy(st + s_tiles.off, p->tiles.data(), s_tiles.bytes);
  if (!need.empty()) memcpy(st + s_need.off, need.data(), s_need.bytes);
  if (!(p->d_plan = dev_alloc<char>(p, sh.plan_bytes))) return p->rc;
  if (!(p->d_in = dev_alloc<char>(p, sh.in_bytes))) return p->rc;
  for (cudaEvent_t* e : {&p->ev_h2d0, &p->ev_h2d1, &p->ev_embed0, &p->ev_embed1, &p->ev_run1})
    PART_CUDA(p, cudaEventCreate(e));
  for (cudaEvent_t* e : {&p->ev_join, &p->ev_bits, &p->ev_rsum, &p->ev_shard})
    PART_CUDA(p, cudaEventCreateWithFlags(e, cudaEventDisableTiming));
  cudaStream_t s0 = dc->stream[0];
  PART_CUDA(p, cudaEventRecord(p->ev_h2d0, s0));
  PART_CUDA(p, cudaMemcpyAsync(p->d_plan, sh.stage_plan, sh.plan_bytes, cudaMemcpyHostToDevice, s0));
  if (seg.total) PART_CUDA(p, cudaMemcpyAsync(d_small, st, seg.total, cudaMemcpyHostToDevice, s0));
  p->info.h2d_bytes = static_cast<int64_t>(sh.plan_bytes + seg.total);
  char* d = p->d_plan;
  char* di = p->d_in;
  p->dcsr.n_samples = sh.N; p->dcsr.nnz = sh.nnz;
  p->dcsr.row_ptr = reinterpret_cast<int64_t*>(di + sh.in_rowptr.off);
  p->dcsr.col = reinterpret_cast<int32_t*>(di + sh.in_col.off);
  p->dcsr.val = sh.need_val ? reinterpret_cast<double*>(di + sh.in_val.off) : nullptr;
  p->dtree.n_nodes = B; p->dtree.height = 0;
  p->dtree.parent = reinterpret_cast<int32_t*>(di + sh.in_parent.off);
  p->dtree.length = reinterpret_cast<double*>(di + sh.in_len.off);
  p->dtree.child_ptr = reinterpret_cast<int32_t*>(di + sh.in_cptr.off);
  p->dtree.child_idx = reinterpret_cast<int32_t*>(di + sh.in_cidx.off);
  p->dtree.level_nodes = reinterpret_cast<int32_t*>(di + sh.in_lvl.off);
  p->dtree.level_parent = reinterpret_cast<int32_t*>(di + sh.in_lpar.off);
  p->d_level_ptr = reinterpret_cast<int32_t*>(di + sh.in_lptr.off);
  p->d_lenf = reinterpret_cast<float*>(di + sh.in_lenf.off);
  p->d_post = sh.unsorted_l ? reinterpret_cast<int32_t*>(di + sh.in_post.off) : nullptr;
  p->d_mult = sh.node_mult ? reinterpret_cast<const double*>(di + sh.in_mult.off) : nullptr;
  p->d_q0 = d + sh.pl_q0.off;
  p->d_q1 = d + sh.pl_hi.off;
  p->d_q2 = d + sh.pl_lo.off;
  p->d_lenq = reinterpret_cast<double*>(d + sh.pl_lenq.off);
  p->d_order = reinterpret_cast<int32_t*>(d + sh.pl_order.off);
  p->d_col_exp = reinterpret_cast<int32_t*>(d + sh.pl_cexp.off);
  p->d_len_col = reinterpret_cast<double*>(d + sh.pl_lcol.off);
  p->d_chunks.end = reinterpret_cast<int32_t*>(d + sh.pl_cend.off);
  p->d_chunks.scale = reinterpret_cast<double*>(d + sh.pl_cscale.off);
  p->d_chunks.n = static_cast<int32_t>(sh.cols.chunk_end.size());
  p->d_chunks.shift = sh.cols.chunk_shift.empty() ? nullptr : reinterpret_cast<int32_t*>(d + sh.pl_cshift.off);
  p->d_chunks.biased = sh.cols.i8 && sh.cols.biased;
  p->d_tiles = reinterpret_cast<Tile*>(d_small + s_tiles.off);
  p->d_need = need.empty() ? nullptr : reinterpret_cast<uint8_t*>(d_small + s_need.off);

  const int chunks = weighted_scratch_chunks(B);
  const bool i8 = sh.cols.i8, intacc = sh.cols.intacc;
  if (sh.exact || sh.weighted) {
    const int64_t per = static_cast<int64_t>(p->shard_nw) * 32;
    p->ws_slab = sh.exact ? sh.np : std::min<int64_t>(per, std::max<int64_t>(kTile, (2LL << 30) / (8LL * B) / kTile * kTile));
    if (!sh.exact && sh.knobs.ws_slab > 0)
      p->ws_slab = std::min<int64_t>(per, round_up(sh.knobs.ws_slab, kTile));
    if (!(p->d_E = dev_alloc<double>(p, static_cast<size_t>(B) * p->ws_slab))) return p->rc;
    if (!(p->d_total = dev_alloc<double>(p, sh.np))) return p->rc;
    if (sh.unsorted_l && !(p->d_list_ptr = dev_alloc<int64_t>(p, sh.N + 2))) return p->rc;
    if (!sh.exact) {
      const size_t a_samples = sh.capacity ? static_cast<size_t>(2 * sh.shards.shard_rows) : static_cast<size_t>(sh.np);
      if (!(p->d_A = dev_alloc<float>(p, static_cast<size_t>(sh.kp) * a_samples))) return p->rc;
      if (sh.keyed && !(p->d_K = dev_alloc<int32_t>(p, static_cast<size_t>(sh.kp) * a_samples))) return p->rc;
      if (sh.capacity) {
        for (int k = 0; k < 2; ++k)
          if (!(p->d_V[k] = dev_alloc<float>(p, static_cast<size_t>(sh.kp) * sh.shards.shard_rows))) return p->rc;
        p->ev_fetch.assign(sh.shards.n_shards, nullptr);
        p->ev_used.assign(sh.shards.n_shards, nullptr);
        for (int k = 0; k < sh.shards.n_shards; ++k) {
          PART_CUDA(p, cudaEventCreateWithFlags(&p->ev_fetch[k], cudaEventDisableTiming));
          PART_CUDA(p, cudaEventCreateWithFlags(&p->ev_used[k], cudaEventDisableTiming));
        }
        unsigned long long* cnts = dev_alloc<unsigned long long>(p, p->cap.size() + 1);
        if (!cnts) return p->rc;
        for (size_t k = 0; k < p->cap.size(); ++k) {
          Part::CapGroup& cb = p->cap[k];
          const size_t cnt = static_cast<size_t>(cb.count);
          cb.cnt = cnts + k;
          if (!(cb.out = dev_alloc<float>(p, cnt))) return p->rc;
          if (!(cb.flagged = dev_alloc<uint32_t>(p, cnt))) return p->rc;
          if (!(cb.n_flagged_host = pin_alloc<unsigned long long>(p, 1))) return p->rc;
          *cb.n_flagged_host = 0;
          if (!(cb.ex.count = pin_alloc<unsigned long long>(p, 1))) return p->rc;
          if (!(cb.ex.index = pin_alloc<int64_t>(p, kMaxExceptions))) return p->rc;
          if (!(cb.ex.value = pin_alloc<double>(p, kMaxExceptions))) return p->rc;
          cb.ex.cap = kMaxExceptions;
          *cb.ex.count = 0;
          PART_CUDA(p, cudaEventCreateWithFlags(&cb.done, cudaEventDisableTiming));
        }
      }
      if (!(p->d_W = dev_alloc<double>(p, sh.np))) return p->rc;
      if (!(p->d_scratch = dev_alloc<double>(p, static_cast<size_t>(chunks) * sh.np))) return p->rc;
      if (!(p->d_flag_counts = dev_alloc<unsigned long long>(p, p->mine.size() + 1))) return p->rc;
      const size_t ws_words = static_cast<size_t>(kFixupCtas) * B * (sh.keyed ? 2 : 1);
      for (int k = 0; k < 2; ++k) {
        if (!(p->d_fix_ws[k] = dev_alloc<long long>(p, ws_words))) return p->rc;
        PART_CUDA(p, cudaMemsetAsync(p->d_fix_ws[k], 0, sizeof(long long) * ws_words, s0));
      }
    }
  } else {
    const size_t words = sh.fused_embed ? static_cast<size_t>(sh.kp) * sh.nw : static_cast<size_t>(B) * sh.nw;
    p->peer_push = sh.exchange == Shared::kNccl && !sh.bits_feed && sh.world <= 8 && sh.knobs.peer_push != 0;
    if (p->peer_push) {
      for (int k = 0; k < 2; ++k) {
        cudaError_t e = cudaSuccess;
        p->d_bits2[k] = static_cast<uint32_t*>(dc->sym.alloc(words * sizeof(uint32_t), &e));
        if (!p->d_bits2[k]) return pfail(p, FRC_ERR_OOM, std::string("symmetric heap: ") + cudaGetErrorString(e));
      }
      bool usable = true;
      if (sym_sync(p, &usable) != FRC_OK) return p->rc;
      if (!usable) p->peer_push = false;
    }
    if (p->peer_push) {
      for (int k = 0; k < 2; ++k) {
        size_t blk = 0;
        for (; blk < dc->sym.blocks.size(); ++blk) {
          char* base = dc->sym.blocks[blk].p;
          if (reinterpret_cast<char*>(p->d_bits2[k]) >= base &&
              reinterpret_cast<char*>(p->d_bits2[k]) < base + dc->sym.blocks[blk].cap) break;
        }
        const size_t off = reinterpret_cast<char*>(p->d_bits2[k]) - dc->sym.blocks[blk].p;
        p->peers[k].n = sh.world; p->peers[k].self = sh.rank0;
        for (int r = 0; r < sh.world; ++r) p->peers[k].p[r] = reinterpret_cast<uint32_t*>(c->sym_peer[blk][r] + off);
      }
      p->d_bits = p->d_bits2[0];
    } else if (!(p->d_bits = dev_alloc<uint32_t>(p, std::max<size_t>(words, 64)))) return p->rc;
    const size_t ns = sh.fused_embed ? static_cast<size_t>(presence_node_scratch_words(B, p->shard_nw)) : 0;
    if (ns && !(p->d_node_scratch = dev_alloc<uint32_t>(p, ns))) return p->rc;
    const size_t opsz = sh.bits_feed ? 256 : static_cast<size_t>(sh.np) * sh.kp * (i8 ? 1 : 2);
    if (!(p->d_P = dev_alloc<char>(p, opsz))) return p->rc;
    if (!(p->d_Bh = dev_alloc<char>(p, opsz))) return p->rc;
    if (!(p->d_Bl = dev_alloc<char>(p, opsz))) return p->rc;
    if (sh.bits_feed && !(p->d_bitsS = dev_alloc<uint32_t>(p, static_cast<size_t>(sh.np) * (sh.kp / 32)))) return p->rc;
    if (!(p->d_r = dev_alloc<double>(p, sh.np))) return p->rc;
    if (!(p->d_scratch = dev_alloc<double>(p, static_cast<size_t>(chunks) * sh.np))) return p->rc;
    if (!(p->d_flag_counts = dev_alloc<unsigned long long>(p, p->mine.size() + 1))) return p->rc;
    if (i8 && !(p->d_flag_u = dev_alloc<double>(p, 1))) return p->rc;
    if (i8 && !(p->d_qerr = dev_alloc<double>(p, sh.kp))) return p->rc;
    if (i8 && !(p->d_qam = dev_alloc<uint32_t>(p, sh.kp))) return p->rc;
    if (intacc && !(p->d_r_int = dev_alloc<long long>(p, sh.np))) return p->rc;
    std::string terr;
    if (sh.bits_feed) {
      p->tc = tc_operands_create_bits(p->d_bitsS, sh.np, sh.kp, static_cast<const uint8_t*>(p->d_q0),
                                      static_cast<const uint8_t*>(p->d_q1), static_cast<const uint8_t*>(p->d_q2),
                                      p->d_chunks, p->d_len_col, p->d_flag_u, p->d_r_int,
                                      std::ldexp(1.0, sh.cols.e_min), &terr);
    } else {
      p->tc = tc_operands_create(p->d_P, p->d_Bh, p->d_Bl, sh.np, sh.kp, i8, p->d_chunks, p->d_len_col, p->d_flag_u, &terr);
      if (p->tc && intacc) tc_operands_set_int(p->tc, p->d_r_int, std::ldexp(1.0, sh.cols.e_min));
    }
    if (!p->tc) return pfail(p, FRC_ERR_CUDA, terr);
    if (i8) {
      p->info.kernel_launches += launch_quantize_lengths(
          p->d_len_col, p->d_col_exp, sh.kp, static_cast<uint8_t*>(p->d_q0), static_cast<uint8_t*>(p->d_q1),
          static_cast<uint8_t*>(p->d_q2), p->d_qam, p->d_lenq, p->d_qerr, p->d_flag_u, s0);
      PART_CUDA(p, cudaGetLastError());
    }
  }
  {
    const int vb = sh.exact ? 8 : 4;
    const int64_t want = std::max<int64_t>(kMinSlots, std::min<int64_t>(kSlots, kSlotBytesBudget / (p->max_band * vb)));
    p->n_slots = static_cast<int>(std::min<int64_t>(want, std::max<int64_t>(2, static_cast<int64_t>(p->mine.size()) + 1)));
  }
  if (p->mine.empty()) p->n_slots = 0;
  for (int k = 0; k < p->n_slots; ++k) {
    Slot& sl = p->slots[k];
    if (sh.exact) {
      if (!(sl.dev64 = dev_alloc<double>(p, p->max_band))) return p->rc;
      if (sh.d2h && !(sl.host64 = pin_alloc<double>(p, p->max_band))) return p->rc;
    } else if (sh.capacity) {
      if (sh.d2h && !(sl.host32 = pin_alloc<float>(p, p->max_band))) return p->rc;
    } else {
      if (!(sl.dev32 = dev_alloc<float>(p, p->max_band))) return p->rc;
      if (sh.d2h && !(sl.host32 = pin_alloc<float>(p, p->max_band))) return p->rc;
      if (!(sl.flagged = dev_alloc<uint32_t>(p, p->max_band))) return p->rc;
      if (!(sl.n_flagged_host = pin_alloc<unsigned long long>(p, 1))) return p->rc;
      *sl.n_flagged_host = 0;
      if (!(sl.ex.count = pin_alloc<unsigned long long>(p, 1))) return p->rc;
      if (!(sl.ex.index = pin_alloc<int64_t>(p, kMaxExceptions))) return p->rc;
      if (!(sl.ex.value = pin_alloc<double>(p, kMaxExceptions))) return p->rc;
      sl.ex.cap = kMaxExceptions;
      *sl.ex.count = 0;
    }
    for (cudaEvent_t* e : {&sl.k0, &sl.k1, &sl.k2, &sl.done}) PART_CUDA(p, cudaEventCreate(e));
  }
  return FRC_OK;
}

int launch_part_stage1(Part* p) {
  const Shared& sh = *p->sh;
  DevCtx* dc = p->dc;
  cudaStream_t s0 = dc->stream[0];
  p->dtree.height = sh.tree_height;
  p->info.tree_height = sh.tree_height;
  PART_CUDA(p, cudaMemcpyAsync(p->d_in, sh.stage_in, sh.in_col.off, cudaMemcpyHostToDevice, s0));
  int64_t up = static_cast<int64_t>(sh.in_col.off);
  const int64_t k0 = p->csr_k0, n = p->csr_k1 - p->csr_k0;
  if (n > 0) {
    PART_CUDA(p, cudaMemcpyAsync(p->d_in + sh.in_col.off + 4 * k0, sh.stage_in + sh.in_col.off + 4 * k0, 4 * n,
                                 cudaMemcpyHostToDevice, s0));
    up += 4 * n;
    if (sh.need_val) {
      PART_CUDA(p, cudaMemcpyAsync(p->d_in + sh.in_val.off + 8 * k0, sh.stage_in + sh.in_val.off + 8 * k0, 8 * n,
                                   cudaMemcpyHostToDevice, s0));
      up += 8 * n;
    }
  }
  p->info.h2d_bytes += up;
  PART_CUDA(p, cudaEventRecord(p->ev_h2d1, s0));
  return embed_stage1(p);
}
int launch_part_stage2(Part* p) {
  if (embed_stage2(p)) return p->rc;
  return start_pairs(p);
}

void aggregate_info(frc_job* j) {
  frc_info_t& a = j->info;
  const Shared& sh = j->sh;
  a = frc_info_t{};
  a.path_taken = sh.exact ? FRC_PATH_EXACT : FRC_PATH_FAST;
  a.n_bands_total = static_cast<int32_t>(sh.bands.size());
  a.tree_height = sh.tree_height;
  a.n_pairs_total = sh.N >= 2 ? tri(sh.N) : 0;
  a.n_nodes_padded = sh.exact ? sh.B : sh.kp;
  a.operand_kind = (!sh.exact && !sh.weighted) ? (sh.cols.i8 ? (sh.bits_feed ? 3 : 2) : 1) : 0;
  a.n_devices = static_cast<int32_t>(j->parts.size());
  a.value_bytes = sh.exact ? 8 : 4;
  a.create_ms = j->create_ms;
  for (auto& p : j->parts) {
    const frc_info_t& i = p->info;
    a.n_bands_mine += static_cast<int32_t>(p->mine.size());
    a.n_pairs_mine += i.n_pairs_mine;
    a.kernel_launches += i.kernel_launches;
    a.h2d_ms = std::max(a.h2d_ms, i.h2d_ms);
    a.embed_ms = std::max(a.embed_ms, i.embed_ms);
    a.pairs_ms += i.pairs_ms;
    a.fixup_ms += i.fixup_ms;
    a.run_ms = std::max(a.run_ms, i.run_ms);
    a.h2d_bytes += i.h2d_bytes;
    a.d2h_bytes += i.d2h_bytes;
    a.embed_bytes += i.embed_bytes;
    a.flagged_pairs += i.flagged_pairs;
    a.gather_bytes += i.gather_bytes;
    a.exceptions += i.exceptions;
  }
}

}

extern "C" {

int frc_create(frc_ctx_t* ctx, const frc_tree_t* tree, const frc_csr_t* abnd, const frc_opts_t* opts,
               frc_job_t** out) {
  g_create_error.clear();
  if (!out) { g_create_error = "frc_create: out is NULL"; return FRC_ERR_ARG; }
  *out = nullptr;
  if (!tree || !abnd || !opts) { g_create_error = "frc_create: NULL argument"; return FRC_ERR_ARG; }
  DeviceGuard guard;
  const auto t_create0 = std::chrono::steady_clock::now();
  frc_job* j = new frc_job();
  Shared& sh = j->sh;
  bool workers_busy = false;
  auto bail = [&](int rc) {
    if (workers_busy) { j->ctx->pool->wait(); workers_busy = false; }
    g_create_error = j->err; destroy_job(j); return rc;
  };
  sh.knobs = Knobs::read();
  const bool trace = sh.knobs.trace;
  auto tp0 = t_create0;
  auto mark = [&](const char* what) {
    if (!trace) return;
    auto now = std::chrono::steady_clock::now();
    fprintf(stderr, "[frc_create] %-32s %8.1f us\n", what, std::chrono::duration<double, std::micro>(now - tp0).count());
    tp0 = now;
  };

  int rc = validate_header(j, tree, abnd, opts);
  if (rc) return bail(rc);
  const int32_t B0 = sh.B;
  const int64_t N = sh.N, nnz = sh.nnz;

  if (ctx) {
    if (ctx->in_use) return bail(fail(j, FRC_ERR_STATE, "context already has a live job"));
    j->ctx = ctx;
  } else {
    if (opts->n_devices > 1 || opts->n_devices < 0) rc = frc_ctx_create_multi(opts->n_devices, opts->devices, &j->ctx);
    else rc = frc_ctx_create(opts->n_devices == 1 && opts->devices ? opts->devices[0] : opts->device, &j->ctx);
    if (rc) { j->err = g_create_error; j->ctx = nullptr; return bail(rc); }
    j->own_ctx = true;
  }
  frc_ctx* c = j->ctx;
  c->in_use = true;
// ... 250 lines not shown
  }
  *out = &sl;
  return FRC_OK;
}

void widen_piece(frc_job* j, const Slot& sl, int64_t band_first, int64_t off, int64_t n) {
  const bool trace = j->sh.knobs.trace;
  const auto t0 = std::chrono::steady_clock::now();
  Pool* pool = j->ctx->pool.get();
  int T = static_cast<int>(std::max<int64_t>(1, std::min<int64_t>(std::min(pool->size(), 16), n / 65536)));
  if (j->sh.knobs.widen_threads > 0) T = std::max(1, std::min(T, j->sh.knobs.widen_threads));
  const float* src = sl.host32 + off;
  double* dst = j->wide;
  constexpr int64_t kChunk = 16384;
  const int64_t n_chunks = (n + kChunk - 1) / kChunk;
  std::atomic<int64_t> next{0};
  std::atomic<int64_t>* nx = &next;
  pool->run(T, [=](int t) {
    for (int64_t ch = t < n_chunks ? t : n_chunks; ch < n_chunks;) {
      const int64_t lo = ch * kChunk, hi = std::min(n, lo + kChunk);
      widen_band(src + lo, dst + lo, hi - lo, false);
      ch = T + nx->fetch_add(1, std::memory_order_relaxed);
    }
  });
  const int64_t n_ex = std::min<int64_t>(static_cast<int64_t>(*sl.ex.count), sl.ex.cap);
  for (int64_t k = 0; k < n_ex; ++k) {
    const int64_t at = sl.ex.index[k] - band_first - off;
    if (at >= 0 && at < n) dst[at] = sl.ex.value[k];
  }
  if (trace)
    fprintf(stderr, "[host] widened %lld pairs on %d threads in %.0f us\n", static_cast<long long>(n), T,
            std::chrono::duration<double, std::micro>(std::chrono::steady_clock::now() - t0).count());
}

int next_chunk(frc_job* j, int mode, const void** data, int64_t* first_index, int64_t* count) {
  const Shared& sh = j->sh;
  *data = nullptr; *first_index = 0; *count = 0;
  if (j->read_mode == 0) j->read_mode = mode;
  if (j->read_mode != mode) return fail(j, FRC_ERR_STATE, "frc_next and frc_next_f32 cannot be mixed on one pass of a job");
  if (mode == 2 && sh.exact)
    return fail(j, FRC_ERR_STATE, "this job took the exact path (bit-exact float64): read it with frc_next");
  if (mode == 1 && !sh.exact && !sh.d2h)
    return fail(j, FRC_ERR_STATE, "FRC_FLAG_NO_D2H on a fast path keeps fp32 in HBM: read it with frc_next_f32");
  DeviceGuard guard;
  if (mode == 1 && j->held_part >= 0 && !sh.exact && j->piece_off < j->piece_end) {
    const int64_t n = std::min(kWidePiece, j->piece_end - j->piece_off);
    widen_piece(j, j->parts[j->held_part]->slots[j->held_slot], j->piece_first, j->piece_off, n);
    *data = j->wide;
    *first_index = j->piece_first + j->piece_off;
    *count = n;
    j->piece_off += n;
    return FRC_OK;
  }
  if (j->held_part >= 0) {
    Part* hp = j->parts[j->held_part].get();
    j->held_part = -1; j->held_slot = -1;
    if (hp->next_enqueue < hp->mine.size()) {
      cudaSetDevice(hp->dc->device);
      if (enqueue_band(hp, hp->next_enqueue)) return fail(j, hp->rc, hp->err);
      ++hp->next_enqueue;
    }
  }
  if (j->next_item >= j->order.size()) return FRC_OK;
  const frc_job::Item it = j->order[j->next_item];
  Part* p = j->parts[it.part].get();
  Slot* sl = nullptr;
  if (part_wait_band(p, static_cast<size_t>(it.idx), &sl)) return fail(j, p->rc, p->err);
  const Band& b = p->bands[it.idx];
  int64_t deliver_n = b.count;
  if (sh.exact) {
    *data = sh.d2h ? sl->host64 : sl->dev64;
  } else if (mode == 2) {
    *data = sh.d2h ? sl->host32 : sl->dev32;
  } else {
    deliver_n = std::min(kWidePiece, b.count);
    j->piece_first = b.first; j->piece_off = deliver_n; j->piece_end = b.count;
    widen_piece(j, *sl, b.first, 0, deliver_n);
    *data = j->wide;
  }
  *first_index = b.first;
  *count = deliver_n;
  j->held_first = b.first; j->held_count = b.count;
  j->held_part = it.part;
  j->held_slot = static_cast<int>(it.idx % p->n_slots);
  ++p->next_deliver;
  ++j->next_item;
  return FRC_OK;
}

}

extern "C" {

int frc_next(frc_job_t* j, const double** data, int64_t* first_index, int64_t* count) {
  if (!j || !data || !first_index || !count) return FRC_ERR_ARG;
  const void* d = nullptr;
  const int rc = next_chunk(j, 1, &d, first_index, count);
  *data = static_cast<const double*>(d);
  return rc;
}

int frc_next_f32(frc_job_t* j, const float** data, int64_t* first_index, int64_t* count) {
  if (!j || !data || !first_index || !count) return FRC_ERR_ARG;
  const void* d = nullptr;
  const int rc = next_chunk(j, 2, &d, first_index, count);
  *data = static_cast<const float*>(d);
  return rc;
}

int frc_chunk_exceptions(frc_job_t* j, const int64_t** index, const double** value, int64_t* count) {
  if (!j || !index || !value || !count) return FRC_ERR_ARG;
  *index = nullptr; *value = nullptr; *count = 0;
  if (j->held_part < 0 || j->sh.exact) return FRC_OK;
  const Slot& sl = j->parts[j->held_part]->slots[j->held_slot];
  const int64_t n = std::min<int64_t>(static_cast<int64_t>(*sl.ex.count), sl.ex.cap);
  if (n == 0) return FRC_OK;
  j->ex_index.clear(); j->ex_value.clear();
  for (int64_t k = 0; k < n; ++k)
    if (sl.ex.index[k] >= j->held_first && sl.ex.index[k] < j->held_first + j->held_count) {
      j->ex_index.push_back(sl.ex.index[k]);
      j->ex_value.push_back(sl.ex.value[k]);
    }
  *index = j->ex_index.data();
  *value = j->ex_value.data();
  *count = static_cast<int64_t>(j->ex_index.size());
  return FRC_OK;
}

int frc_restart(frc_job_t* j) {
  if (!j) return FRC_ERR_ARG;
  DeviceGuard guard;
  for (auto& p : j->parts) {
    cudaSetDevice(p->dc->device);
    for (auto s : p->dc->stream)
      if (cudaStreamSynchronize(s) != cudaSuccess) return fail(j, FRC_ERR_CUDA, std::string("cudaStreamSynchronize: ") + cudaGetErrorString(cudaGetLastError()));
    p->info.kernel_launches = 0;
  }
  j->next_item = 0;
  j->held_part = j->held_slot = -1;
  j->read_mode = 0;
  j->piece_off = j->piece_end = 0;
  int rc = for_parts(j, embed_stage1);
  if (rc) return rc;
  return for_parts(j, launch_part_stage2);
}

int frc_job_info(const frc_job_t* cj, frc_info_t* info) {
  if (!cj || !info) return FRC_ERR_ARG;
  frc_job* j = const_cast<frc_job*>(cj);
  DeviceGuard guard;
  for (auto& p : j->parts) {
    if (!p->embed_timed && p->ev_embed1) {
      cudaSetDevice(p->dc->device);
      if (cudaEventSynchronize(p->ev_embed1) == cudaSuccess) {
        float a = 0.f, b = 0.f;
        if (cudaEventElapsedTime(&a, p->ev_h2d0, p->ev_h2d1) == cudaSuccess) p->info.h2d_ms = a;
        if (cudaEventElapsedTime(&b, p->ev_embed0, p->ev_embed1) == cudaSuccess) p->info.embed_ms = b;
        p->embed_timed = true;
      }
      cudaGetLastError();
    }
  }
  aggregate_info(j);
  *info = j->info;
  return FRC_OK;
}

void frc_destroy(frc_job_t* j) {
  DeviceGuard guard;
  destroy_job(j);
}

int64_t frc_plan_bands(int64_t n_samples, int64_t band_rows, int32_t rank, int32_t world, uint32_t flags,
                       int64_t* first_index, int64_t* count, int64_t cap) {
  if (world <= 0) { world = 1; rank = 0; }
  if (n_samples < 0 || band_rows < 0 || rank < 0 || rank >= world) return -FRC_ERR_ARG;
  const Knobs knobs = Knobs::read();
  const std::vector<Band> bands = make_bands(n_samples, band_rows, world, !(flags & FRC_FLAG_NO_D2H), knobs.bands_per_rank, 8);
  int64_t n = 0;
  for (const Band& b : bands)
    if (b.owner == rank) {
      if (n < cap && first_index && count) { first_index[n] = b.first; count[n] = b.count; }
      ++n;
    }
  return n;
}

}
```

frackyfrac_b200/csrc/ptx.cuh:

```cuda
#pragma once
#include <cuda.h>
#include <cstdint>

namespace frc {
namespace ptx {

__device__ __forceinline__ uint32_t smem_u32(const void* p) {
  return static_cast<uint32_t>(__cvta_generic_to_shared(p));
}

__device__ __forceinline__ bool elect_one() {
  uint32_t pred = 0;
  asm volatile(
      "{\n\t.reg .pred P;\n\t"
      "elect.sync _|P, 0xffffffff;\n\t"
      "selp.b32 %0, 1, 0, P;\n\t}"
      : "=r"(pred));
  return pred != 0;
}

__device__ __forceinline__ void mbar_init(uint32_t bar, uint32_t count) {
  asm volatile("mbarrier.init.shared::cta.b64 [%0], %1;" ::"r"(bar), "r"(count) : "memory");
}
__device__ __forceinline__ void fence_barrier_init() {
// ... 69 lines not shown
      "cp.async.bulk.tensor.2d.cta_group::2.shared::cluster.global.mbarrier::complete_tx::bytes"
      " [%0], [%1, {%3, %4}], [%2];"
      ::"r"(dst), "l"(reinterpret_cast<uint64_t>(map)), "r"(bar), "r"(c0), "r"(c1)
      : "memory");
}

__device__ __forceinline__ void bulk_load_1d(uint32_t dst, const void* src, uint32_t bytes, uint32_t bar) {
  asm volatile(
      "cp.async.bulk.shared::cluster.global.mbarrier::complete_tx::bytes [%0], [%1], %2, [%3];"
      ::"r"(dst), "l"(reinterpret_cast<uint64_t>(src)), "r"(bytes), "r"(bar)
      : "memory");
}

template <int N>
__device__ __forceinline__ void setmaxnreg_inc() { asm volatile("setmaxnreg.inc.sync.aligned.u32 %0;" ::"n"(N)); }
template <int N>
__device__ __forceinline__ void setmaxnreg_dec() { asm volatile("setmaxnreg.dec.sync.aligned.u32 %0;" ::"n"(N)); }

template <int CG>
__device__ __forceinline__ void tmem_alloc(uint32_t dst_smem, uint32_t ncols) {
  if constexpr (CG == 1)
    asm volatile("tcgen05.alloc.cta_group::1.sync.aligned.shared::cta.b32 [%0], %1;" ::"r"(dst_smem),
                 "r"(ncols) : "memory");
  else
    asm volatile("tcgen05.alloc.cta_group::2.sync.aligned.shared::cta.b32 [%0], %1;" ::"r"(dst_smem),
                 "r"(ncols) : "memory");
}
template <int CG>
__device__ __forceinline__ void tmem_relinquish() {
  if constexpr (CG == 1)
    asm volatile("tcgen05.relinquish_alloc_permit.cta_group::1.sync.aligned;" ::: "memory");
  else
    asm volatile("tcgen05.relinquish_alloc_permit.cta_group::2.sync.aligned;" ::: "memory");
}
template <int CG>
__device__ __forceinline__ void tmem_dealloc(uint32_t taddr, uint32_t ncols) {
  if constexpr (CG == 1)
    asm volatile("tcgen05.dealloc.cta_group::1.sync.aligned.b32 %0, %1;" ::"r"(taddr), "r"(ncols)
                 : "memory");
  else
    asm volatile("tcgen05.dealloc.cta_group::2.sync.aligned.b32 %0, %1;" ::"r"(taddr), "r"(ncols)
                 : "memory");
}
__device__ __forceinline__ void tc_fence_before() {
  asm volatile("tcgen05.fence::before_thread_sync;" ::: "memory");
}
__device__ __forceinline__ void tc_fence_after() {
  asm volatile("tcgen05.fence::after_thread_sync;" ::: "memory");
}

template <int CG>
__device__ __forceinline__ void umma_bf16(uint32_t d_tmem, uint64_t a_desc, uint64_t b_desc,
                                          uint32_t idesc, uint32_t accumulate) {
  if constexpr (CG == 1)
    asm volatile(
        "{\n\t.reg .pred p;\n\t"
        "setp.ne.b32 p, %4, 0;\n\t"
        "tcgen05.mma.cta_group::1.kind::f16 [%0], %1, %2, %3, p;\n\t}"
        ::"r"(d_tmem), "l"(a_desc), "l"(b_desc), "r"(idesc), "r"(accumulate) : "memory");
  else
    asm volatile(
        "{\n\t.reg .pred p;\n\t"
        "setp.ne.b32 p, %4, 0;\n\t"
        "tcgen05.mma.cta_group::2.kind::f16 [%0], %1, %2, %3, p;\n\t}"
        ::"r"(d_tmem), "l"(a_desc), "l"(b_desc), "r"(idesc), "r"(accumulate) : "memory");
}

template <int CG>
__device__ __forceinline__ void umma_i8(uint32_t d_tmem, uint64_t a_desc, uint64_t b_desc,
                                        uint32_t idesc, uint32_t accumulate) {
  if constexpr (CG == 1)
    asm volatile(
        "{\n\t.reg .pred p;\n\t"
        "setp.ne.b32 p, %4, 0;\n\t"
        "tcgen05.mma.cta_group::1.kind::i8 [%0], %1, %2, %3, p;\n\t}"
        ::"r"(d_tmem), "l"(a_desc), "l"(b_desc), "r"(idesc), "r"(accumulate) : "memory");
  else
    asm volatile(
        "{\n\t.reg .pred p;\n\t"
        "setp.ne.b32 p, %4, 0;\n\t"
        "tcgen05.mma.cta_group::2.kind::i8 [%0], %1, %2, %3, p;\n\t}"
        ::"r"(d_tmem), "l"(a_desc), "l"(b_desc), "r"(idesc), "r"(accumulate) : "memory");
}

__device__ __forceinline__ void umma_commit(uint32_t bar) {
  asm volatile("tcgen05.commit.cta_group::1.mbarrier::arrive::one.shared::cluster.b64 [%0];" ::"r"(bar)
               : "memory");
}
__device__ __forceinline__ void umma_commit_2sm(uint32_t bar, uint16_t mask) {
  asm volatile(
      "tcgen05.commit.cta_group::2.mbarrier::arrive::one.shared::cluster.multicast::cluster.b64"
      " [%0], %1;" ::"r"(bar), "h"(mask) : "memory");
}

__device__ __forceinline__ void tmem_ld_32x32(uint32_t taddr, uint32_t (&v)[32]) {
  asm volatile(
      "tcgen05.ld.sync.aligned.32x32b.x32.b32 "
      "{%0, %1, %2, %3, %4, %5, %6, %7, %8, %9, %10, %11, %12, %13, %14, %15, "
      "%16, %17, %18, %19, %20, %21, %22, %23, %24, %25, %26, %27, %28, %29, %30, %31}, [%32];"
      : "=r"(v[0]), "=r"(v[1]), "=r"(v[2]), "=r"(v[3]), "=r"(v[4]), "=r"(v[5]), "=r"(v[6]),
        "=r"(v[7]), "=r"(v[8]), "=r"(v[9]), "=r"(v[10]), "=r"(v[11]), "=r"(v[12]), "=r"(v[13]),
        "=r"(v[14]), "=r"(v[15]), "=r"(v[16]), "=r"(v[17]), "=r"(v[18]), "=r"(v[19]), "=r"(v[20]),
        "=r"(v[21]), "=r"(v[22]), "=r"(v[23]), "=r"(v[24]), "=r"(v[25]), "=r"(v[26]), "=r"(v[27]),
        "=r"(v[28]), "=r"(v[29]), "=r"(v[30]), "=r"(v[31])
      : "r"(taddr)
      : "memory");
}
__device__ __forceinline__ void tmem_ld_32x16(uint32_t taddr, uint32_t (&v)[16]) {
  asm volatile(
      "tcgen05.ld.sync.aligned.32x32b.x16.b32 "
      "{%0, %1, %2, %3, %4, %5, %6, %7, %8, %9, %10, %11, %12, %13, %14, %15}, [%16];"
      : "=r"(v[0]), "=r"(v[1]), "=r"(v[2]), "=r"(v[3]), "=r"(v[4]), "=r"(v[5]), "=r"(v[6]),
        "=r"(v[7]), "=r"(v[8]), "=r"(v[9]), "=r"(v[10]), "=r"(v[11]), "=r"(v[12]), "=r"(v[13]),
        "=r"(v[14]), "=r"(v[15])
      : "r"(taddr)
      : "memory");
}
__device__ __forceinline__ void tmem_ld_32x8(uint32_t taddr, uint32_t (&v)[8]) {
  asm volatile(
      "tcgen05.ld.sync.aligned.32x32b.x8.b32 {%0, %1, %2, %3, %4, %5, %6, %7}, [%8];"
      : "=r"(v[0]), "=r"(v[1]), "=r"(v[2]), "=r"(v[3]), "=r"(v[4]), "=r"(v[5]), "=r"(v[6]), "=r"(v[7])
      : "r"(taddr)
      : "memory");
}
__device__ __forceinline__ void tmem_ld_wait() {
  asm volatile("tcgen05.wait::ld.sync.aligned;" ::: "memory");
}

__device__ __forceinline__ uint64_t umma_desc_k_sw128(uint32_t smem_addr) {
  uint64_t d = 0;
  d |= static_cast<uint64_t>((smem_addr & 0x3FFFF) >> 4);
  d |= static_cast<uint64_t>(1) << 16;
  d |= static_cast<uint64_t>(1024 >> 4) << 32;
  d |= static_cast<uint64_t>(1) << 46;
  d |= static_cast<uint64_t>(2) << 61;
  return d;
}
__host__ __device__ constexpr uint32_t umma_idesc_bf16(int m, int n) {
  return (1u << 4)
         | (1u << 7)
         | (1u << 10)
         | (static_cast<uint32_t>(n >> 3) << 17)
         | (static_cast<uint32_t>(m >> 4) << 24);
}

__host__ __device__ constexpr uint32_t umma_idesc_u8(int m, int n) {
  return (2u << 4)
         | (0u << 7)
         | (0u << 10)
         | (static_cast<uint32_t>(n >> 3) << 17)
         | (static_cast<uint32_t>(m >> 4) << 24);
}

__device__ __forceinline__ uint32_t cluster_ctarank() {
  uint32_t r;
  asm volatile("mov.u32 %0, %%cluster_ctarank;" : "=r"(r));
  return r;
}
__device__ __forceinline__ void cluster_sync_all() {
  asm volatile("barrier.cluster.arrive.release;\n\tbarrier.cluster.wait.acquire;" ::: "memory");
}

}
}
```

frackyfrac_b200/csrc/unweighted_tc.cu:

```cuda
#include <cuda.h>
#include <cuda_runtime.h>

#include <cstdio>
#include <cstdlib>
#include <type_traits>

#include "frc_internal.h"
#include "ptx.cuh"
#include "wire.cuh"

namespace frc {

namespace {

constexpr int BM = 128, BN = 128, BK = 64, UK = 16;
constexpr int A_BYTES = BM * BK * 2;
constexpr int B_BYTES = BN * BK * 2;
constexpr int EPI_WARP0 = 2;
constexpr int DN = 2 * BN;
constexpr uint32_t TMEM_COLS = 2 * DN;

constexpr int STAGES2 = 6;
constexpr int STAGE2_BYTES = A_BYTES + B_BYTES;
constexpr int NUM_BARS2 = 2 * STAGES2 + 4;
constexpr int SMEM2_BYTES = STAGES2 * STAGE2_BYTES + NUM_BARS2 * 8 + 16 + 1024;
constexpr int BKB = 128;
#ifdef FRC_TC_TIMELINE
__device__ unsigned long long g_tc_dbg[512 * 8];
__device__ unsigned long long g_bits_dbg[512 * 8];
#define TL(x) x
#define TL_ON(mask) ((dbg & (mask)) != 0)
#else
#define TL(x)
#define TL_ON(mask) false
#endif
constexpr int EPI2_WARPS = 16;
constexpr int EPI2_COLS = 128 / (EPI2_WARPS / 4);
constexpr int THREADS2 = 32 * (EPI_WARP0 + EPI2_WARPS);

__device__ __forceinline__ void drain_int(uint32_t taddr, uint32_t shift, unsigned long long (&acc)[EPI2_COLS]) {
  const uint32_t m0 = 1u << shift, m1 = 256u << shift;
  uint32_t v[2][8], w[2][8];
  ptx::tmem_ld_32x8(taddr, v[0]);
  ptx::tmem_ld_32x8(taddr + BN, w[0]);
#pragma unroll
  for (int cc = 0; cc < EPI2_COLS / 8; ++cc) {
    ptx::tmem_ld_wait();
    if (cc + 1 < EPI2_COLS / 8) {
      ptx::tmem_ld_32x8(taddr + (cc + 1) * 8, v[(cc + 1) & 1]);
      ptx::tmem_ld_32x8(taddr + BN + (cc + 1) * 8, w[(cc + 1) & 1]);
    }
#pragma unroll
    for (int x = 0; x < 8; ++x)
      acc[cc * 8 + x] += static_cast<unsigned long long>(v[cc & 1][x]) * m1 +
                         static_cast<unsigned long long>(w[cc & 1][x]) * m0;
  }
}

__device__ __forceinline__ void ratio_int(const unsigned long long (&acc)[EPI2_COLS], const long long* __restrict__ r_int,
                                          int64_t i0, int64_t j, int lane, int64_t n_samples, int64_t off,
                                          long long flag_u_int, float* __restrict__ out, uint32_t* __restrict__ flagged,
                                          unsigned long long* __restrict__ n_flagged) {
  const long long rj = j < n_samples ? r_int[j] : 0;
  const long long ri_lane = r_int[i0 + lane];
#pragma unroll
  for (int n0 = 0; n0 < EPI2_COLS; n0 += 8) {
    float dv[8];
    bool fu[8];
#pragma unroll
    for (int x = 0; x < 8; ++x) {
      const long long ri = __shfl_sync(0xffffffffu, ri_lane, n0 + x);
      const long long sh = static_cast<long long>(acc[n0 + x]);
      const unsigned long long U = static_cast<unsigned long long>(ri + rj - 2 * sh);
      const unsigned long long V = U + static_cast<unsigned long long>(sh);
      const float Uf = fmaf(__uint2float_rn(static_cast<uint32_t>(U >> 32)), 4294967296.f,
                            __uint2float_rn(static_cast<uint32_t>(U)));
      const float Vf = fmaf(__uint2float_rn(static_cast<uint32_t>(V >> 32)), 4294967296.f,
                            __uint2float_rn(static_cast<uint32_t>(V)));
      dv[x] = __fdividef(Uf, Vf);
      fu[x] = static_cast<long long>(U) < flag_u_int;
    }
#pragma unroll
    for (int x = 0; x < 8; ++x) {
      const int64_t i = i0 + n0 + x;
      if (i < n_samples && j < i) {
        out[off] = dv[x];
        if (fu[x]) {
          unsigned long long slot = atomicAdd(n_flagged, 1ULL);
          flagged[slot] = static_cast<uint32_t>(off);
        }
      }
      off += i;
    }
  }
}

template <int kMode>
__global__ void __cluster_dims__(2, 1, 1) __launch_bounds__(THREADS2, 1)
k_unweighted_tc2(const __grid_constant__ CUtensorMap mapP, const __grid_constant__ CUtensorMap mapBh,
                 const __grid_constant__ CUtensorMap mapBl, const int32_t* __restrict__ chunk_end,
                 const double* __restrict__ chunk_scale, const int32_t* __restrict__ chunk_shift,
                 int32_t n_chunks, int32_t biased, const double* __restrict__ r,
                 const long long* __restrict__ r_int, double unit, const Tile* __restrict__ tiles, int32_t n_tiles,
                 int64_t n_samples, int64_t first, float* __restrict__ out, double flag_below,
                 const double* __restrict__ flag_u_ptr, uint32_t* __restrict__ flagged,
                 unsigned long long* __restrict__ n_flagged, int dbg) {
  (void)dbg;
  constexpr bool kI8 = kMode != 0;
  constexpr bool kInt = kMode == 2;
  extern __shared__ uint8_t smem_raw[];
  const uint32_t raw = ptx::smem_u32(smem_raw);
  const uint32_t pad = ((raw + 1023u) & ~1023u) - raw;
  uint8_t* smem = smem_raw + pad;
  const uint32_t smem_base = raw + pad;
  const uint32_t bar_base = smem_base + STAGES2 * STAGE2_BYTES;
  auto full_bar = [&](int s) { return bar_base + 8u * s; };
  auto empty_bar = [&](int s) { return bar_base + 8u * (STAGES2 + s); };
  auto tfull_bar = [&](int b) { return bar_base + 8u * (2 * STAGES2 + b); };
  auto tempty_bar = [&](int b) { return bar_base + 8u * (2 * STAGES2 + 2 + b); };
  volatile uint32_t* tmem_slot =
      reinterpret_cast<volatile uint32_t*>(smem + STAGES2 * STAGE2_BYTES + NUM_BARS2 * 8);

  const int warp = threadIdx.x >> 5;
  const int lane = threadIdx.x & 31;
  const uint32_t cta = ptx::cluster_ctarank();
  const int pair = blockIdx.x >> 1;
  const int n_pairs = gridDim.x >> 1;

  if (warp == 0 && lane == 0) {
    ptx::prefetch_tensormap(&mapP);
    ptx::prefetch_tensormap(cta == 0 ? &mapBh : &mapBl);
    for (int s = 0; s < STAGES2; ++s) {
      ptx::mbar_init(full_bar(s), 1);
      ptx::mbar_init(empty_bar(s), 1);
    }
    for (int b = 0; b < 2; ++b) {
      ptx::mbar_init(tfull_bar(b), 1);
      ptx::mbar_init(tempty_bar(b), 2 * EPI2_WARPS);
    }
    ptx::fence_barrier_init();
    ptx::fence_proxy_async();
  }
  if (warp == 1) {
    ptx::tmem_alloc<2>(ptx::smem_u32(const_cast<uint32_t*>(tmem_slot)), TMEM_COLS);
    ptx::tmem_relinquish<2>();
  }
  ptx::tc_fence_before();
  ptx::cluster_sync_all();
  ptx::tc_fence_after();
  const uint32_t tmem_base = *tmem_slot;

  const int n_kblocks = chunk_end[n_chunks - 1];

  if (warp == 0) {
    if (lane == 0) {
      int stage = 0;
      uint32_t phase = 0;
      const void* mapB = cta == 0 ? static_cast<const void*>(&mapBh) : static_cast<const void*>(&mapBl);
      constexpr int kElems = kI8 ? BKB : BKB / 2;
      TL(long long w_empty = 0;)
      for (int t = pair; t < n_tiles; t += n_pairs) {
        const Tile tile = tiles[t];
        const int row_a = (tile.tj + static_cast<int>(cta)) * BM, row_b = tile.ti * BN;
        for (int kb = 0; kb < n_kblocks; ++kb) {
          TL(const long long c0 = clock64();)
          ptx::mbar_wait(empty_bar(stage), phase ^ 1u);
          TL(w_empty += clock64() - c0;)
          const uint32_t sa = smem_base + stage * STAGE2_BYTES;
          if (cta == 0)
            ptx::mbar_expect_tx(full_bar(stage), 2 * ((TL_ON(2) ? 0 : A_BYTES) + (TL_ON(1) ? 0 : B_BYTES)));
          const uint32_t lead_bar = ptx::mapa_u32(full_bar(stage), 0);
          if (!TL_ON(2)) ptx::tma_load_2d_2sm(sa, &mapP, lead_bar, kb * kElems, row_a);
          if (!TL_ON(1)) ptx::tma_load_2d_2sm(sa + A_BYTES, mapB, lead_bar, kb * kElems, row_b);
          if (++stage == STAGES2) { stage = 0; phase ^= 1u; }
        }
      }
      TL(g_tc_dbg[blockIdx.x * 8 + 3] = w_empty;)
    }
    __syncwarp();
  } else if (warp == 1) {
    if (lane == 0 && cta == 0) {
      constexpr uint32_t idesc = kI8 ? ptx::umma_idesc_u8(2 * BM, DN) : ptx::umma_idesc_bf16(2 * BM, DN);
      int stage = 0;
      uint32_t phase = 0;
      uint32_t chunk = 0;
      TL(long long w_tempty = 0; long long w_full = 0; const long long c_start = clock64();)
      for (int t = pair; t < n_tiles; t += n_pairs) {
        int kb = 0;
        for (int ch = 0; ch < n_chunks; ++ch, ++chunk) {
          const uint32_t buf = chunk & 1u;
          TL(const long long c0 = clock64();)
          ptx::mbar_wait(tempty_bar(buf), ((chunk >> 1) & 1u) ^ 1u);
          TL(w_tempty += clock64() - c0;)
          ptx::tc_fence_after();
          const uint32_t d_tmem = tmem_base + buf * DN;
          const int kb_begin = kb, kb_end = chunk_end[ch];
          for (; kb < kb_end; ++kb) {
            TL(const long long c1 = clock64();)
            ptx::mbar_wait(full_bar(stage), phase);
            TL(w_full += clock64() - c1;)
            ptx::tc_fence_after();
            const uint32_t sa = smem_base + stage * STAGE2_BYTES;
            const uint64_t da = ptx::umma_desc_k_sw128(sa);
            const uint64_t db = ptx::umma_desc_k_sw128(sa + A_BYTES);
#pragma unroll
            for (int k = 0; k < 4; ++k) {
              const uint32_t accum = (kb > kb_begin || k > 0) ? 1u : 0u;
              if constexpr (kI8) ptx::umma_i8<2>(d_tmem, da + 2u * k, db + 2u * k, idesc, accum);
              else ptx::umma_bf16<2>(d_tmem, da + 2u * k, db + 2u * k, idesc, accum);
            }
            ptx::umma_commit_2sm(empty_bar(stage), 3);
            if (++stage == STAGES2) { stage = 0; phase ^= 1u; }
          }
          ptx::umma_commit_2sm(tfull_bar(buf), 3);
        }
      }
      TL(g_tc_dbg[blockIdx.x * 8 + 0] = w_tempty; g_tc_dbg[blockIdx.x * 8 + 1] = w_full;
         g_tc_dbg[blockIdx.x * 8 + 2] = clock64() - c_start;)
    }
    __syncwarp();
  } else {
    const int q = warp & 3;
    const int cg = (warp - EPI_WARP0) >> 2;
    using Acc = typename std::conditional<kInt, unsigned long long,
                                          typename std::conditional<kI8, double, float>::type>::type;
    const float flag_u = flag_u_ptr ? static_cast<float>(*flag_u_ptr) : 0.f;
    const float flag_d = static_cast<float>(flag_below);
    const long long flag_u_int = (kInt && flag_u_ptr) ? static_cast<long long>(*flag_u_ptr / unit) : 0;
    double acc0 = 0.0;
    if constexpr (kI8 && !kInt)
      if (biased) for (int ch = 0; ch < n_chunks; ++ch) acc0 -= 4503599627370496.0 * chunk_scale[ch];
    uint32_t chunk = 0;
    TL(long long w_tfull = 0; long long t_drain = 0; long long t_ratio = 0; const long long e_start = clock64();)
    for (int t = pair; t < n_tiles; t += n_pairs) {
      const Tile tile = tiles[t];
      Acc acc[EPI2_COLS];
#pragma unroll
      for (int n = 0; n < EPI2_COLS; ++n) acc[n] = static_cast<Acc>(acc0);
      for (int ch = 0; ch < n_chunks; ++ch, ++chunk) {
        const uint32_t buf = chunk & 1u;
        const double scale = (kI8 && !kInt) ? chunk_scale[ch] : 1.0;
        const uint32_t shift = kInt ? static_cast<uint32_t>(chunk_shift[ch]) : 0u;
        TL(const long long c0 = clock64();)
        ptx::mbar_wait(tfull_bar(buf), (chunk >> 1) & 1u);
        TL(const long long c1 = clock64();)
        ptx::tc_fence_after();
        const uint32_t taddr = tmem_base + (static_cast<uint32_t>(q * 32) << 16) + buf * DN + cg * EPI2_COLS;
        if constexpr (kInt) {
          drain_int(taddr, shift, acc);
        } else if constexpr (kI8) {
          auto drain = [&](auto kBiased) {
            uint32_t v[2][8], w[2][8];
            ptx::tmem_ld_32x8(taddr, v[0]);
            ptx::tmem_ld_32x8(taddr + BN, w[0]);
#pragma unroll
            for (int cc = 0; cc < EPI2_COLS / 8; ++cc) {
              ptx::tmem_ld_wait();
              if (cc + 1 < EPI2_COLS / 8) {
                ptx::tmem_ld_32x8(taddr + (cc + 1) * 8, v[(cc + 1) & 1]);
                ptx::tmem_ld_32x8(taddr + BN + (cc + 1) * 8, w[(cc + 1) & 1]);
              }
#pragma unroll
              for (int x = 0; x < 8; ++x) {
                const unsigned long long S = static_cast<unsigned long long>(v[cc & 1][x]) * 256ull + w[cc & 1][x];
                double D = __longlong_as_double(static_cast<long long>(S | 0x4330000000000000ull));
                if (!decltype(kBiased)::value) D -= 4503599627370496.0;
                acc[cc * 8 + x] = fma(scale, D, acc[cc * 8 + x]);
              }
            }
          };
          if (biased) drain(std::true_type{}); else drain(std::false_type{});
        } else {
#pragma unroll
          for (int cc = 0; cc < EPI2_COLS / 16; ++cc) {
            uint32_t v[16], w[16];
            ptx::tmem_ld_32x16(taddr + cc * 16, v);
            ptx::tmem_ld_32x16(taddr + BN + cc * 16, w);
            ptx::tmem_ld_wait();
#pragma unroll
            for (int x = 0; x < 16; ++x) acc[cc * 16 + x] += __uint_as_float(v[x]) + __uint_as_float(w[x]);
          }
        }
        ptx::tc_fence_before();
        __syncwarp();
        if (lane == 0) ptx::mbar_arrive_cluster(tempty_bar(buf), 0);
        TL(w_tfull += c1 - c0; t_drain += clock64() - c1;)
      }
      TL(const long long c2 = clock64();)
      const int64_t j = static_cast<int64_t>(tile.tj + static_cast<int>(cta)) * BM + q * 32 + lane;
      const int64_t i0 = static_cast<int64_t>(tile.ti) * BN + cg * EPI2_COLS;
      static_assert(EPI2_COLS == 32, "r[i] is broadcast from lane n");
      if (TL_ON(4)) {
        if (acc[0] == static_cast<Acc>(-1.5)) out[0] = 0.f;
      } else if (static_cast<int64_t>(tile.tj + static_cast<int>(cta)) * BM + q * 32 < i0 + EPI2_COLS) {
        int64_t off = i0 * (i0 - 1) / 2 - first + j;
        if constexpr (kInt) {
          ratio_int(acc, r_int, i0, j, lane, n_samples, off, flag_u_int, out, flagged, n_flagged);
        } else {
          const double rj = j < n_samples ? r[j] : 0.0;
          const double ri_lane = r[i0 + lane];
#pragma unroll
          for (int n0 = 0; n0 < EPI2_COLS; n0 += 8) {
            float dv[8], uv[8];
#pragma unroll
            for (int x = 0; x < 8; ++x) {
              const double ri = __shfl_sync(0xffffffffu, ri_lane, n0 + x);
              const double sd = static_cast<double>(acc[n0 + x]);
              const double U = fma(-2.0, sd, ri + rj);
              uv[x] = static_cast<float>(U);
              dv[x] = __fdividef(uv[x], uv[x] + static_cast<float>(sd));
            }
#pragma unroll
            for (int x = 0; x < 8; ++x) {
              const int64_t i = i0 + n0 + x;
              if (i < n_samples && j < i) {
                out[off] = dv[x];
                if (dv[x] < flag_d || uv[x] < flag_u) {
                  unsigned long long slot = atomicAdd(n_flagged, 1ULL);
                  flagged[slot] = static_cast<uint32_t>(off);
                }
              }
              off += i;
            }
          }
        }
      }
      TL(t_ratio += clock64() - c2;)
    }
    TL(if (warp == EPI_WARP0 && lane == 0) {
      g_tc_dbg[blockIdx.x * 8 + 4] = w_tfull;
      g_tc_dbg[blockIdx.x * 8 + 5] = t_drain;
      g_tc_dbg[blockIdx.x * 8 + 6] = t_ratio;
      g_tc_dbg[blockIdx.x * 8 + 7] = clock64() - e_start;
    })
  }

  ptx::tc_fence_before();
  ptx::cluster_sync_all();
  if (warp == 1) {
    __syncwarp();
    ptx::tmem_dealloc<2>(tmem_base, TMEM_COLS);
  }
}

namespace bits {
constexpr int OSTAGES = 5;
constexpr int OSTAGE_BYTES = A_BYTES + B_BYTES;
constexpr int BSTAGES = 8;
constexpr int BITS_TILE = 128 * 16;
constexpr int BSTAGE_BYTES = 2 * BITS_TILE + 2 * BKB;
constexpr int NUM_BARS = 3 * OSTAGES + 2 * BSTAGES + 4;
constexpr int SMEM_BYTES = OSTAGES * OSTAGE_BYTES + BSTAGES * BSTAGE_BYTES + NUM_BARS * 8 + 16 + 1024;
constexpr int PROD_WARP0 = 4, PROD_WARPS = 8;
constexpr int EPI_WARP0 = 12;
constexpr int THREADS = 32 * (EPI_WARP0 + EPI2_WARPS);

__device__ __forceinline__ uint32_t mask4(uint32_t nib) {
  uint32_t m;
  asm("prmt.b32 %0, %1, 0, 0xBA98;" : "=r"(m) : "r"(nib * 0x10204080u));
  return m;
}
}

__global__ void __cluster_dims__(2, 1, 1) __launch_bounds__(bits::THREADS, 1)
k_unweighted_bits2(const __grid_constant__ CUtensorMap mapBits, const uint8_t* __restrict__ qa,
                   const uint8_t* __restrict__ qh, const uint8_t* __restrict__ ql,
                   const int32_t* __restrict__ chunk_end, const int32_t* __restrict__ chunk_shift,
                   int32_t n_chunks, const long long* __restrict__ r_int, double unit,
                   const Tile* __restrict__ tiles, int32_t n_tiles, int64_t n_samples, int64_t first,
                   float* __restrict__ out, const double* __restrict__ flag_u_ptr,
                   uint32_t* __restrict__ flagged, unsigned long long* __restrict__ n_flagged) {
  using namespace bits;
  extern __shared__ uint8_t smem_raw[];
  const uint32_t raw = ptx::smem_u32(smem_raw);
  const uint32_t pad = ((raw + 1023u) & ~1023u) - raw;
  uint8_t* smem = smem_raw + pad;
  const uint32_t smem_base = raw + pad;
  const uint32_t bits_base = smem_base + OSTAGES * OSTAGE_BYTES;
  const uint32_t bar_base = bits_base + BSTAGES * BSTAGE_BYTES;
  auto ofull_bar = [&](int s) { return bar_base + 8u * s; };
  auto oempty_bar = [&](int s) { return bar_base + 8u * (OSTAGES + s); };
  auto bfull_bar = [&](int s) { return bar_base + 8u * (2 * OSTAGES + s); };
  auto bempty_bar = [&](int s) { return bar_base + 8u * (2 * OSTAGES + BSTAGES + s); };
  auto tfull_bar = [&](int b) { return bar_base + 8u * (2 * OSTAGES + 2 * BSTAGES + b); };
  auto tempty_bar = [&](int b) { return bar_base + 8u * (2 * OSTAGES + 2 * BSTAGES + 2 + b); };
  auto pfull_bar = [&](int s) { return bar_base + 8u * (2 * OSTAGES + 2 * BSTAGES + 4 + s); };
  volatile uint32_t* tmem_slot = reinterpret_cast<volatile uint32_t*>(
      smem + OSTAGES * OSTAGE_BYTES + BSTAGES * BSTAGE_BYTES + NUM_BARS * 8);

  const int warp = threadIdx.x >> 5;
  const int lane = threadIdx.x & 31;
  const uint32_t cta = ptx::cluster_ctarank();
  const int pair = blockIdx.x >> 1;
  const int n_pairs = gridDim.x >> 1;

  if (warp == 0 && lane == 0) {
    ptx::prefetch_tensormap(&mapBits);
    for (int s = 0; s < OSTAGES; ++s) {
      ptx::mbar_init(ofull_bar(s), PROD_WARPS + 1);
      ptx::mbar_init(oempty_bar(s), 1);
      ptx::mbar_init(pfull_bar(s), PROD_WARPS);
    }
    for (int s = 0; s < BSTAGES; ++s) {
      ptx::mbar_init(bfull_bar(s), 1);
      ptx::mbar_init(bempty_bar(s), PROD_WARPS);
    }
    for (int b = 0; b < 2; ++b) {
      ptx::mbar_init(tfull_bar(b), 1);
      ptx::mbar_init(tempty_bar(b), 2 * EPI2_WARPS);
    }
    ptx::fence_barrier_init();
    ptx::fence_proxy_async();
  }
  if (warp == 1) {
    ptx::tmem_alloc<2>(ptx::smem_u32(const_cast<uint32_t*>(tmem_slot)), TMEM_COLS);
    ptx::tmem_relinquish<2>();
  }
  ptx::tc_fence_before();
  ptx::cluster_sync_all();
  ptx::tc_fence_after();
  const uint32_t tmem_base = *tmem_slot;
  const int n_kblocks = chunk_end[n_chunks - 1];

  if (warp == 0) {
    ptx::setmaxnreg_dec<24>();
    if (lane == 0) {
      int stage = 0;
      uint32_t phase = 0;
      const uint8_t* qb = cta == 0 ? qh : ql;
      for (int t = pair; t < n_tiles; t += n_pairs) {
        const Tile tile = tiles[t];
        const int row_a = (tile.tj + static_cast<int>(cta)) * BM, row_b = tile.ti * BN;
        for (int kb = 0; kb < n_kblocks; ++kb) {
          TL(const long long c0 = clock64();)
          ptx::mbar_wait(bempty_bar(stage), phase ^ 1u);
          TL(g_bits_dbg[blockIdx.x * 8 + 0] += clock64() - c0;)
          const uint32_t sb = bits_base + stage * BSTAGE_BYTES;
          ptx::mbar_expect_tx(bfull_bar(stage), BSTAGE_BYTES);
          ptx::tma_load_2d(sb, &mapBits, bfull_bar(stage), kb * 16, row_a);
          ptx::tma_load_2d(sb + BITS_TILE, &mapBits, bfull_bar(stage), kb * 16, row_b);
          ptx::bulk_load_1d(sb + 2 * BITS_TILE, qa + static_cast<int64_t>(kb) * BKB, BKB, bfull_bar(stage));
          ptx::bulk_load_1d(sb + 2 * BITS_TILE + BKB, qb + static_cast<int64_t>(kb) * BKB, BKB, bfull_bar(stage));
          if (++stage == BSTAGES) { stage = 0; phase ^= 1u; }
        }
      }
    }
    __syncwarp();
  } else if (warp == 1) {
    ptx::setmaxnreg_dec<24>();
    if (lane == 0 && cta == 0) {
      constexpr uint32_t idesc = ptx::umma_idesc_u8(2 * BM, DN);
      int stage = 0;
      uint32_t phase = 0;
      uint32_t chunk = 0;
      for (int t = pair; t < n_tiles; t += n_pairs) {
        int kb = 0;
        for (int ch = 0; ch < n_chunks; ++ch, ++chunk) {
          const uint32_t buf = chunk & 1u;
          TL(const long long c0 = clock64();)
          ptx::mbar_wait(tempty_bar(buf), ((chunk >> 1) & 1u) ^ 1u);
          TL(g_bits_dbg[blockIdx.x * 8 + 1] += clock64() - c0;)
          ptx::tc_fence_after();
          const uint32_t d_tmem = tmem_base + buf * DN;
          const int kb_begin = kb, kb_end = chunk_end[ch];
          for (; kb < kb_end; ++kb) {
            TL(const long long c1 = clock64();)
            ptx::mbar_wait(ofull_bar(stage), phase);
            TL(g_bits_dbg[blockIdx.x * 8 + 2] += clock64() - c1;)
            ptx::tc_fence_after();
            const uint32_t sa = smem_base + stage * OSTAGE_BYTES;
            const uint64_t da = ptx::umma_desc_k_sw128(sa);
            const uint64_t db = ptx::umma_desc_k_sw128(sa + A_BYTES);
#pragma unroll
            for (int k = 0; k < 4; ++k)
              ptx::umma_i8<2>(d_tmem, da + 2u * k, db + 2u * k, idesc, (kb > kb_begin || k > 0) ? 1u : 0u);
            ptx::umma_commit_2sm(oempty_bar(stage), 3);
            if (++stage == OSTAGES) { stage = 0; phase ^= 1u; }
          }
          ptx::umma_commit_2sm(tfull_bar(buf), 3);
        }
      }
    }
    __syncwarp();
  } else if (warp < PROD_WARP0) {
    ptx::setmaxnreg_dec<24>();
    if (warp == 2 && cta == 1 && lane == 0) {
      int stage = 0;
      uint32_t phase = 0;
      for (int t = pair; t < n_tiles; t += n_pairs)
        for (int kb = 0; kb < n_kblocks; ++kb) {
          ptx::mbar_wait(pfull_bar(stage), phase);
          ptx::mbar_arrive_cluster_relaxed(ofull_bar(stage), 0);
          if (++stage == OSTAGES) { stage = 0; phase ^= 1u; }
        }
    }
// ... 149 lines not shown
    }
    if (lane == 0) store_fixed(out, off, uniq / (uniq + comm), first, ex);
  }
}

typedef CUresult (*PFN_tmapEncodeTiled)(CUtensorMap*, CUtensorMapDataType, cuuint32_t, void*,
                                        const cuuint64_t*, const cuuint64_t*, const cuuint32_t*,
                                        const cuuint32_t*, CUtensorMapInterleave, CUtensorMapSwizzle,
                                        CUtensorMapL2promotion, CUtensorMapFloatOOBfill);
PFN_tmapEncodeTiled g_encode = nullptr;

bool make_map(CUtensorMap* m, const void* base, int64_t rows, int32_t kp, int box_rows, bool i8,
              std::string* err) {
  const int esz = i8 ? 1 : 2;
  cuuint64_t dims[2] = {static_cast<cuuint64_t>(kp), static_cast<cuuint64_t>(rows)};
  cuuint64_t strides[1] = {static_cast<cuuint64_t>(kp) * esz};
  cuuint32_t box[2] = {static_cast<cuuint32_t>(BKB / esz), static_cast<cuuint32_t>(box_rows)};
  cuuint32_t estr[2] = {1, 1};
  CUresult rc = g_encode(m, i8 ? CU_TENSOR_MAP_DATA_TYPE_UINT8 : CU_TENSOR_MAP_DATA_TYPE_BFLOAT16, 2,
                         const_cast<void*>(base), dims, strides, box, estr, CU_TENSOR_MAP_INTERLEAVE_NONE,
                         CU_TENSOR_MAP_SWIZZLE_128B, CU_TENSOR_MAP_L2_PROMOTION_L2_256B,
                         CU_TENSOR_MAP_FLOAT_OOB_FILL_NONE);
  if (rc != CUDA_SUCCESS) {
    if (err) *err = "cuTensorMapEncodeTiled failed with CUresult " + std::to_string(static_cast<int>(rc));
    return false;
  }
  return true;
}

}

struct TcOperands {
  bool from_bits = false;
  CUtensorMap mapP, mapBh, mapBl;
  const void* P = nullptr;
  CUtensorMap mapBits;
  const uint32_t* bitsS = nullptr;
  const uint8_t *qa = nullptr, *qh = nullptr, *ql = nullptr;
  bool i8;
  int32_t kp;
  TcChunks chunks;
  const double* len_col;
  const double* flag_u;
  const long long* r_int = nullptr;
  double unit = 1.0;
  int dbg = 0;
};

bool tc_setup(std::string* err) {
  if (!g_encode) {
    void* fn = nullptr;
    cudaDriverEntryPointQueryResult q;
    cudaError_t e = cudaGetDriverEntryPoint("cuTensorMapEncodeTiled", &fn, cudaEnableDefault, &q);
    if (e != cudaSuccess || q != cudaDriverEntryPointSuccess || !fn) {
      if (err) *err = "cuTensorMapEncodeTiled is not available from the driver";
      return false;
    }
    g_encode = reinterpret_cast<PFN_tmapEncodeTiled>(fn);
  }
  cudaError_t e = cudaFuncSetAttribute(k_unweighted_tc2<0>, cudaFuncAttributeMaxDynamicSharedMemorySize, SMEM2_BYTES);
  if (e == cudaSuccess)
    e = cudaFuncSetAttribute(k_unweighted_tc2<1>, cudaFuncAttributeMaxDynamicSharedMemorySize, SMEM2_BYTES);
  if (e == cudaSuccess)
    e = cudaFuncSetAttribute(k_unweighted_tc2<2>, cudaFuncAttributeMaxDynamicSharedMemorySize, SMEM2_BYTES);
  if (e != cudaSuccess) {
    if (err) *err = std::string("cudaFuncSetAttribute(k_unweighted_tc2): ") + cudaGetErrorString(e);
    return false;
  }
  e = cudaFuncSetAttribute(k_unweighted_bits2, cudaFuncAttributeMaxDynamicSharedMemorySize, bits::SMEM_BYTES);
  if (e != cudaSuccess) {
    if (err) *err = std::string("cudaFuncSetAttribute(k_unweighted_bits2): ") + cudaGetErrorString(e);
    return false;
  }
  return true;
}

TcOperands* tc_operands_create(const void* P, const void* Bh, const void* Bl, int64_t np, int32_t kp,
                               bool i8, const TcChunks& chunks, const double* len_col, const double* flag_u,
                               std::string* err) {
  if (!g_encode) { if (err) *err = "tc_setup has not run on this device context"; return nullptr; }
  TcOperands* o = new TcOperands();
  if (const char* de = getenv("FRC_TC_DEBUG")) o->dbg = atoi(de);
  o->P = P;
  o->i8 = i8;
  o->kp = kp;
  o->chunks = chunks;
  o->len_col = len_col;
  o->flag_u = flag_u;
  if (!make_map(&o->mapP, P, np, kp, BM, i8, err) || !make_map(&o->mapBh, Bh, np, kp, BN, i8, err) ||
      !make_map(&o->mapBl, Bl, np, kp, BN, i8, err)) {
    delete o;
    return nullptr;
  }
  return o;
}
TcOperands* tc_operands_create_bits(const uint32_t* bitsS, int64_t np, int32_t kp, const uint8_t* qa,
                                    const uint8_t* qh, const uint8_t* ql, const TcChunks& chunks,
                                    const double* len_col, const double* flag_u, const long long* r_int,
                                    double unit, std::string* err) {
  if (!g_encode) { if (err) *err = "tc_setup has not run on this device context"; return nullptr; }
  TcOperands* o = new TcOperands();
  o->from_bits = true;
  o->bitsS = bitsS; o->qa = qa; o->qh = qh; o->ql = ql;
  o->i8 = true; o->kp = kp; o->chunks = chunks;
  o->len_col = len_col; o->flag_u = flag_u; o->r_int = r_int; o->unit = unit;
  cuuint64_t dims[2] = {static_cast<cuuint64_t>(kp / 8), static_cast<cuuint64_t>(np)};
  cuuint64_t strides[1] = {static_cast<cuuint64_t>(kp / 8)};
  cuuint32_t box[2] = {16, 128};
  cuuint32_t estr[2] = {1, 1};
  CUresult rc = g_encode(&o->mapBits, CU_TENSOR_MAP_DATA_TYPE_UINT8, 2, const_cast<uint32_t*>(bitsS), dims, strides,
                         box, estr, CU_TENSOR_MAP_INTERLEAVE_NONE, CU_TENSOR_MAP_SWIZZLE_NONE,
                         CU_TENSOR_MAP_L2_PROMOTION_L2_128B, CU_TENSOR_MAP_FLOAT_OOB_FILL_NONE);
  if (rc != CUDA_SUCCESS) {
    if (err) *err = "cuTensorMapEncodeTiled(bits) failed with CUresult " + std::to_string(static_cast<int>(rc));
    delete o;
    return nullptr;
  }
  return o;
}
void tc_operands_set_int(TcOperands* o, const long long* r_int, double unit) { o->r_int = r_int; o->unit = unit; }
void tc_operands_destroy(TcOperands* o) { delete o; }

}
extern "C" int frc_debug_tc_counters(unsigned long long* out, int n) {
#ifdef FRC_TC_TIMELINE
  if (n > 512 * 8) n = 512 * 8;
  return static_cast<int>(cudaMemcpyFromSymbol(out, frc::g_tc_dbg, sizeof(unsigned long long) * n));
#else
  (void)out; (void)n;
  return -1;
#endif
}
extern "C" int frc_debug_bits_counters(unsigned long long* out, int n, int clear) {
#ifdef FRC_TC_TIMELINE
  if (n > 512 * 8) n = 512 * 8;
  int rc = static_cast<int>(cudaMemcpyFromSymbol(out, frc::g_bits_dbg, sizeof(unsigned long long) * n));
  if (clear) { static unsigned long long z[512 * 8] = {0}; cudaMemcpyToSymbol(frc::g_bits_dbg, z, sizeof(z)); }
  return rc;
#else
  (void)out; (void)n; (void)clear;
  return -1;
#endif
}
namespace frc {

int tc_chunk_kblocks() {
  const char* e = getenv("FRC_TC_CHUNK_KBLOCKS");
  int x = e ? atoi(e) : 64;
  return x < 1 ? 1 : x;
}

int launch_unweighted_tc(const TcOperands* ops, const double* r, const Tile* tiles, int32_t n_tiles,
                         int64_t n_samples, int64_t first, float* out, double flag_below,
                         uint32_t* flagged, unsigned long long* n_flagged, int num_sms, cudaStream_t s) {
  if (n_tiles <= 0) return 0;
  const int pairs = num_sms / 2;
  const int grid = 2 * (n_tiles < pairs ? n_tiles : pairs);
  const TcChunks& c = ops->chunks;
  if (ops->from_bits) {
    k_unweighted_bits2<<<grid, bits::THREADS, bits::SMEM_BYTES, s>>>(
        ops->mapBits, ops->qa, ops->qh, ops->ql, c.end, c.shift, c.n, ops->r_int, ops->unit, tiles, n_tiles, n_samples,
        first, out, ops->flag_u, flagged, n_flagged);
    return 1;
  }
#define FRC_TC2_ARGS ops->mapP, ops->mapBh, ops->mapBl, c.end, c.scale, c.shift, c.n, c.biased ? 1 : 0, r, ops->r_int, \
                     ops->unit, tiles, n_tiles, n_samples, first, out, flag_below, ops->flag_u, flagged, n_flagged, ops->dbg
  if (ops->i8 && ops->r_int) k_unweighted_tc2<2><<<grid, THREADS2, SMEM2_BYTES, s>>>(FRC_TC2_ARGS);
  else if (ops->i8) k_unweighted_tc2<1><<<grid, THREADS2, SMEM2_BYTES, s>>>(FRC_TC2_ARGS);
  else k_unweighted_tc2<0><<<grid, THREADS2, SMEM2_BYTES, s>>>(FRC_TC2_ARGS);
#undef FRC_TC2_ARGS
  return 1;
}

int launch_unweighted_fixup(const TcOperands* ops, const uint32_t* flagged, const unsigned long long* n_flagged,
                            unsigned long long* count_host, int64_t first, float* out, const Exceptions& ex,
                            int num_sms, cudaStream_t s) {
  const auto kernel = ops->from_bits ? k_unweighted_fixup<Rows::kBits>
                      : ops->i8      ? k_unweighted_fixup<Rows::kU8>
                                     : k_unweighted_fixup<Rows::kBf16>;
  const void* rows = ops->from_bits ? static_cast<const void*>(ops->bitsS) : ops->P;
  kernel<<<num_sms * 4, 256, 0, s>>>(rows, ops->kp, ops->len_col, flagged, n_flagged, count_host, first, out, ex);
  return 1;
}

}
```

Measured before the change: 30.76 billion.

## Overlap operand expansion with tensor-core GEMM via PDL and per-kblock ready counters

```diff
diff --git a/frackyfrac_b200/csrc/embed.cu b/frackyfrac_b200/csrc/embed.cu
--- a/frackyfrac_b200/csrc/embed.cu
+++ b/frackyfrac_b200/csrc/embed.cu
@@ -1,4 +1,5 @@
 #include "frc_internal.h"
+#include "ptx.cuh"
 
 namespace frc {
 
@@ -447,59 +448,73 @@
                      const uint8_t* __restrict__ ql, uint8_t* __restrict__ A, uint8_t* __restrict__ Bh,
                      uint8_t* __restrict__ Bl, const uint8_t* __restrict__ need,
                      const uint32_t* __restrict__ qam, const int32_t* __restrict__ col_exp, int32_t e_min,
-                     long long* __restrict__ r_int) {
+                     long long* __restrict__ r_int, uint32_t* __restrict__ ready,
+                     unsigned long long* __restrict__ stamps) {
   __shared__ __align__(16) uint32_t words[8][128];
   __shared__ __align__(16) uint32_t sq[128];
-  const int32_t v0 = blockIdx.x * 128;
-  const int32_t w0 = blockIdx.y * 8;
-  const uint32_t nd = need ? need[blockIdx.y] : 3u;
-  if (nd == 0u) return;
-  for (int idx = threadIdx.x; idx < 1024; idx += 256) {
-    int word = idx >> 7, node = idx & 127;
-    uint32_t x = 0;
-    if (w0 + word < nw) x = bitsT[static_cast<int64_t>(w0 + word) * kp + v0 + node];
-    words[word][node] = x;
-  }
-  if (r_int != nullptr && threadIdx.x < 128) sq[threadIdx.x] = qam[v0 + threadIdx.x];
-  __syncthreads();
-  const int wi = threadIdx.x >> 5, lane = threadIdx.x & 31;
-  const int32_t va = v0 + 4 * lane;
-  const uint4 w4 = *reinterpret_cast<const uint4*>(&words[wi][4 * lane]);
-  const uint32_t a4 = *reinterpret_cast<const uint32_t*>(qa + va);
-  const uint32_t h4 = *reinterpret_cast<const uint32_t*>(qh + va);
-  const uint32_t l4 = *reinterpret_cast<const uint32_t*>(ql + va);
-  const int64_t s0 = (static_cast<int64_t>(w0) + wi) * 32;
+  ptx::griddep_launch_dependents();
+  const int32_t n_groups = static_cast<int32_t>((np + 255) / 256), n_kb = kp / 128;
+  const int32_t kb = static_cast<int32_t>(blockIdx.x) / n_groups, grp = static_cast<int32_t>(blockIdx.x) - kb * n_groups;
+  if (ready != nullptr && blockIdx.x == 0 && threadIdx.x == 0) stamps[0] = ptx::globaltimer();
+  const int32_t v0 = kb * 128;
+  const int32_t w0 = grp * 8;
+  const uint32_t nd = need ? need[grp] : 3u;
+  if (nd != 0u) {
+    for (int idx = threadIdx.x; idx < 1024; idx += 256) {
+      int word = idx >> 7, node = idx & 127;
+      uint32_t x = 0;
+      if (w0 + word < nw) x = bitsT[static_cast<int64_t>(w0 + word) * kp + v0 + node];
+      words[word][node] = x;
+    }
+    if (r_int != nullptr && threadIdx.x < 128) sq[threadIdx.x] = qam[v0 + threadIdx.x];
+    __syncthreads();
+    const int wi = threadIdx.x >> 5, lane = threadIdx.x & 31;
+    const int32_t va = v0 + 4 * lane;
+    const uint4 w4 = *reinterpret_cast<const uint4*>(&words[wi][4 * lane]);
+    const uint32_t a4 = *reinterpret_cast<const uint32_t*>(qa + va);
+    const uint32_t h4 = *reinterpret_cast<const uint32_t*>(qh + va);
+    const uint32_t l4 = *reinterpret_cast<const uint32_t*>(ql + va);
+    const int64_t s0 = (static_cast<int64_t>(w0) + wi) * 32;
 #pragma unroll 4
-  for (int it = 0; it < 32; ++it) {
-    const int64_t s = s0 + it;
-    if (s >= np) break;
-    const uint32_t bits = ((w4.x >> it) & 1u) | (((w4.y >> it) & 1u) << 8) | (((w4.z >> it) & 1u) << 16) |
-                          (((w4.w >> it) & 1u) << 24);
-    const uint32_t m = bits * 0xFFu;
-    const int64_t o = s * kp + va;
-    if (nd & 1u) *reinterpret_cast<uint32_t*>(A + o) = a4 & m;
-    if (nd & 2u) {
-      *reinterpret_cast<uint32_t*>(Bh + o) = h4 & m;
-      *reinterpret_cast<uint32_t*>(Bl + o) = l4 & m;
-    }
-  }
-  if (r_int != nullptr) {
-    const uint32_t m = 1u << lane;
-    uint32_t a0 = 0, a1 = 0, a2 = 0, a3 = 0;
+    for (int it = 0; it < 32; ++it) {
+      const int64_t s = s0 + it;
+      if (s >= np) break;
+      const uint32_t bits = ((w4.x >> it) & 1u) | (((w4.y >> it) & 1u) << 8) | (((w4.z >> it) & 1u) << 16) |
+                            (((w4.w >> it) & 1u) << 24);
+      const uint32_t m = bits * 0xFFu;
+      const int64_t o = s * kp + va;
+      if (nd & 1u) *reinterpret_cast<uint32_t*>(A + o) = a4 & m;
+      if (nd & 2u) {
+        *reinterpret_cast<uint32_t*>(Bh + o) = h4 & m;
+        *reinterpret_cast<uint32_t*>(Bl + o) = l4 & m;
+      }
+    }
+    if (r_int != nullptr) {
+      const uint32_t m = 1u << lane;
+      uint32_t a0 = 0, a1 = 0, a2 = 0, a3 = 0;
 #pragma unroll 8
-    for (int k = 0; k < 128; k += 4) {
-      const uint4 w = *reinterpret_cast<const uint4*>(&words[wi][k]);
-      const uint4 q = *reinterpret_cast<const uint4*>(&sq[k]);
-      a0 += (w.x & m) ? q.x : 0u;
-      a1 += (w.y & m) ? q.y : 0u;
-      a2 += (w.z & m) ? q.z : 0u;
-      a3 += (w.w & m) ? q.w : 0u;
-    }
-    const uint32_t sum = (a0 + a1) + (a2 + a3);
-    const int64_t s = s0 + lane;
-    if (sum != 0u && s < np)
-      atomicAdd(reinterpret_cast<unsigned long long*>(r_int) + s,
-                static_cast<unsigned long long>(sum) << (col_exp[v0] - e_min));
+      for (int k = 0; k < 128; k += 4) {
+        const uint4 w = *reinterpret_cast<const uint4*>(&words[wi][k]);
+        const uint4 q = *reinterpret_cast<const uint4*>(&sq[k]);
+        a0 += (w.x & m) ? q.x : 0u;
+        a1 += (w.y & m) ? q.y : 0u;
+        a2 += (w.z & m) ? q.z : 0u;
+        a3 += (w.w & m) ? q.w : 0u;
+      }
+      const uint32_t sum = (a0 + a1) + (a2 + a3);
+      const int64_t s = s0 + lane;
+      if (sum != 0u && s < np)
+        atomicAdd(reinterpret_cast<unsigned long long*>(r_int) + s,
+                  static_cast<unsigned long long>(sum) << (col_exp[v0] - e_min));
+    }
+  }
+  if (ready != nullptr) {
+    ptx::fence_proxy_async_global();
+    __syncthreads();
+    if (threadIdx.x == 0) {
+      ptx::red_release_add(ready + kb, 1u);
+      if (ptx::atom_release_add(ready + n_kb, 1u) + 1u == gridDim.x) stamps[1] = ptx::globaltimer();
+    }
   }
 }
 
@@ -677,6 +692,7 @@
 
 void embed_setup() {
   cudaFuncSetAttribute(k_embed_presence_fused<true>, cudaFuncAttributeMaxDynamicSharedMemorySize, 200 * 1024);
+  cudaFuncSetAttribute(k_expand_operands_u8, cudaFuncAttributePreferredSharedMemoryCarveout, cudaSharedmemCarveoutMaxShared);
 }
 
 int64_t presence_node_scratch_words(int32_t n_nodes, int32_t nw) {
@@ -725,14 +741,14 @@
 int launch_expand_operands_t(const uint32_t* bitsT, int32_t nw, int32_t kp, int64_t np, bool i8,
                              const void* q0, const void* q1, const void* q2, void* P, void* Bh, void* Bl,
                              const uint8_t* need, const uint32_t* qam, const int32_t* col_exp, int32_t e_min,
-                             long long* r_int, cudaStream_t s) {
+                             long long* r_int, uint32_t* ready, unsigned long long* stamps, cudaStream_t s) {
   if (i8) {
-    if (r_int) cudaMemsetAsync(r_int, 0, sizeof(long long) * np, s);
-    dim3 grid(kp / 128, static_cast<unsigned>((np + 255) / 256));
+    const unsigned grid = static_cast<unsigned>(kp / 128) * static_cast<unsigned>((np + 255) / 256);
     k_expand_operands_u8<<<grid, 256, 0, s>>>(bitsT, nw, kp, np, static_cast<const uint8_t*>(q0),
                                               static_cast<const uint8_t*>(q1), static_cast<const uint8_t*>(q2),
                                               static_cast<uint8_t*>(P), static_cast<uint8_t*>(Bh),
-                                              static_cast<uint8_t*>(Bl), need, qam, col_exp, e_min, r_int);
+                                              static_cast<uint8_t*>(Bl), need, qam, col_exp, e_min, r_int, ready,
+                                              stamps);
   } else {
     (void)q0;
     dim3 grid(kp / 64, static_cast<unsigned>((np + 255) / 256));
diff --git a/frackyfrac_b200/csrc/frc_internal.h b/frackyfrac_b200/csrc/frc_internal.h
--- a/frackyfrac_b200/csrc/frc_internal.h
+++ b/frackyfrac_b200/csrc/frc_internal.h
@@ -81,7 +81,7 @@
 int launch_expand_operands_t(const uint32_t* bitsT, int32_t nw, int32_t kp, int64_t np, bool i8,
                              const void* q0, const void* q1, const void* q2, void* P, void* Bh, void* Bl,
                              const uint8_t* need, const uint32_t* qam, const int32_t* col_exp, int32_t e_min,
-                             long long* r_int, cudaStream_t s);
+                             long long* r_int, uint32_t* ready, unsigned long long* stamps, cudaStream_t s);
 int launch_quantize_lengths(const double* len_col, const int32_t* col_exp, int32_t kp, uint8_t* qa,
                             uint8_t* qh, uint8_t* ql, uint32_t* qam, double* lenq, double* qerr, double* flag_u,
                             cudaStream_t s);
@@ -143,7 +143,8 @@
 int tc_chunk_kblocks();
 int launch_unweighted_tc(const TcOperands* ops, const double* r, const Tile* tiles, int32_t n_tiles,
                          int64_t n_samples, int64_t first, float* out, double flag_below,
-                         uint32_t* flagged, unsigned long long* n_flagged, int num_sms, cudaStream_t s);
+                         uint32_t* flagged, unsigned long long* n_flagged, int num_sms, cudaStream_t s,
+                         const uint32_t* ready, uint32_t ready_target);
 int launch_unweighted_fixup(const TcOperands* ops, const uint32_t* flagged,
                             const unsigned long long* n_flagged, unsigned long long* count_host,
                             int64_t first, float* out, const Exceptions& ex, int num_sms, cudaStream_t s);
diff --git a/frackyfrac_b200/csrc/job.cu b/frackyfrac_b200/csrc/job.cu
--- a/frackyfrac_b200/csrc/job.cu
+++ b/frackyfrac_b200/csrc/job.cu
@@ -242,6 +242,9 @@
   int32_t* d_level_ptr = nullptr;
   int32_t* d_post = nullptr;
   unsigned long long* d_flag_counts = nullptr;
+  size_t n_zeroed = 0;
+  uint32_t* d_ready = nullptr;
+  unsigned long long* h_stamps = nullptr;
   int64_t ws_slab = 0;
   bool peer_push = false;
   uint32_t* d_bits2[2] = {nullptr, nullptr};
@@ -276,6 +279,7 @@
   cudaEvent_t ev_h2d0 = nullptr, ev_h2d1 = nullptr, ev_embed0 = nullptr, ev_embed1 = nullptr;
   cudaEvent_t ev_run1 = nullptr, ev_join = nullptr, ev_bits = nullptr, ev_rsum = nullptr;
   cudaEvent_t ev_shard = nullptr;
+  cudaEvent_t ev_expand = nullptr;
   bool run_timed = false, embed_timed = false;
   std::chrono::steady_clock::time_point t_host0;
 };
@@ -443,8 +447,7 @@
   cudaStream_t s = dc->stream[0];
   int launches = 0;
   p->t_host0 = std::chrono::steady_clock::now();
-  if (p->d_flag_counts)
-    PART_CUDA(p, cudaMemsetAsync(p->d_flag_counts, 0, sizeof(unsigned long long) * (p->mine.size() + 1), s));
+  if (p->d_flag_counts) PART_CUDA(p, cudaMemsetAsync(p->d_flag_counts, 0, sizeof(unsigned long long) * p->n_zeroed, s));
   PART_CUDA(p, cudaEventRecord(p->ev_embed0, s));
   p->info.gather_bytes = 0;
   const bool inproc = sh.exchange == Shared::kInProcess;
@@ -557,10 +560,14 @@
   if (!sh.exact && !sh.weighted) {
     if (sh.fused_embed) {
       const bool rowsum_in_expand = sh.cols.intacc && !sh.bits_feed;
+      if (p->d_ready) {
+        PART_CUDA(p, cudaEventRecord(p->ev_embed1, s));
+        if (!p->mine.empty()) PART_CUDA(p, cudaEventRecord(p->slots[0].k0, s));
+      }
       if (!sh.bits_feed)
         launches += launch_expand_operands_t(p->d_bits, sh.nw, sh.kp, sh.np, sh.cols.i8, p->d_q0, p->d_q1, p->d_q2,
                                              p->d_P, p->d_Bh, p->d_Bl, p->d_need, p->d_qam, p->d_col_exp, sh.cols.e_min,
-                                             rowsum_in_expand ? p->d_r_int : nullptr, s);
+                                             rowsum_in_expand ? p->d_r_int : nullptr, p->d_ready, p->h_stamps, s);
       if (sh.exchange == Shared::kNone) {
         if (!rowsum_in_expand) {
           PART_CUDA(p, cudaEventRecord(p->ev_rsum, dc->stream[1]));
@@ -580,8 +587,10 @@
     }
   }
   PART_CUDA(p, cudaGetLastError());
-  PART_CUDA(p, cudaEventRecord(p->ev_embed1, s));
-  PART_CUDA(p, cudaStreamWaitEvent(dc->stream[1], p->ev_embed1, 0));
+  if (!p->d_ready) {
+    PART_CUDA(p, cudaEventRecord(p->ev_embed1, s));
+    PART_CUDA(p, cudaStreamWaitEvent(dc->stream[1], p->ev_embed1, 0));
+  }
   p->info.kernel_launches += launches;
   p->embed_timed = false;
   return FRC_OK;
@@ -619,7 +628,8 @@
     }
     return FRC_OK;
   }
-  PART_CUDA(p, cudaEventRecord(sl.k0, s));
+  const bool behind_expand = idx == 0 && p->d_ready != nullptr;
+  if (!behind_expand) PART_CUDA(p, cudaEventRecord(sl.k0, s));
   if (sh.exact) {
     if (sh.unsorted_l)
       launches += launch_unsorted_pairs(p->d_list_ptr, p->d_list_id, p->d_list_val, p->dtree.length, b.first, b.count,
@@ -640,7 +650,12 @@
                                         sl.dev32, sl.ex, s, p->d_K, sh.kp);
     } else {
       launches += launch_unweighted_tc(p->tc, p->d_r, p->d_tiles + b.tile_off, b.n_tiles, sh.N, b.first, sl.dev32,
-                                       kFlagBelow, sl.flagged, cnt, dc->num_sms, s);
+                                       kFlagBelow, sl.flagged, cnt, dc->num_sms, s, behind_expand ? p->d_ready : nullptr,
+                                       static_cast<uint32_t>((sh.np + 255) / 256));
+      if (behind_expand) {
+        PART_CUDA(p, cudaEventRecord(p->ev_expand, s));
+        PART_CUDA(p, cudaStreamWaitEvent(dc->stream[1], p->ev_expand, 0));
+      }
       PART_CUDA(p, cudaEventRecord(sl.k1, s));
       launches += launch_unweighted_fixup(p->tc, sl.flagged, cnt, sl.n_flagged_host, b.first, sl.dev32, sl.ex,
                                           dc->num_sms, s);
@@ -730,6 +745,7 @@
   p->info.exceptions = 0;
   p->info.d2h_bytes = 0;
   if (p->mine.empty()) {
+    if (p->d_ready) PART_CUDA(p, cudaEventRecord(p->ev_expand, p->dc->stream[0]));
     PART_CUDA(p, cudaEventRecord(p->ev_run1, p->dc->stream[0]));
     return FRC_OK;
   }
@@ -755,7 +771,7 @@
     if (sl.done) cudaEventDestroy(sl.done);
   }
   for (cudaEvent_t e : {p->ev_h2d0, p->ev_h2d1, p->ev_embed0, p->ev_embed1, p->ev_run1, p->ev_join, p->ev_bits,
-                        p->ev_rsum, p->ev_shard})
+                        p->ev_rsum, p->ev_shard, p->ev_expand})
     if (e) cudaEventDestroy(e);
   for (cudaEvent_t e : p->ev_fetch) if (e) cudaEventDestroy(e);
   for (cudaEvent_t e : p->ev_used) if (e) cudaEventDestroy(e);
@@ -1167,7 +1183,7 @@
   if (!(p->d_in = dev_alloc<char>(p, sh.in_bytes))) return p->rc;
   for (cudaEvent_t* e : {&p->ev_h2d0, &p->ev_h2d1, &p->ev_embed0, &p->ev_embed1, &p->ev_run1})
     PART_CUDA(p, cudaEventCreate(e));
-  for (cudaEvent_t* e : {&p->ev_join, &p->ev_bits, &p->ev_rsum, &p->ev_shard})
+  for (cudaEvent_t* e : {&p->ev_join, &p->ev_bits, &p->ev_rsum, &p->ev_shard, &p->ev_expand})
     PART_CUDA(p, cudaEventCreateWithFlags(e, cudaEventDisableTiming));
   cudaStream_t s0 = dc->stream[0];
   PART_CUDA(p, cudaEventRecord(p->ev_h2d0, s0));
@@ -1249,7 +1265,8 @@
       }
       if (!(p->d_W = dev_alloc<double>(p, sh.np))) return p->rc;
       if (!(p->d_scratch = dev_alloc<double>(p, static_cast<size_t>(chunks) * sh.np))) return p->rc;
-      if (!(p->d_flag_counts = dev_alloc<unsigned long long>(p, p->mine.size() + 1))) return p->rc;
+      p->n_zeroed = p->mine.size() + 1;
+      if (!(p->d_flag_counts = dev_alloc<unsigned long long>(p, p->n_zeroed))) return p->rc;
       const size_t ws_words = static_cast<size_t>(kFixupCtas) * B * (sh.keyed ? 2 : 1);
       for (int k = 0; k < 2; ++k) {
         if (!(p->d_fix_ws[k] = dev_alloc<long long>(p, ws_words))) return p->rc;
@@ -1292,11 +1309,19 @@
     if (sh.bits_feed && !(p->d_bitsS = dev_alloc<uint32_t>(p, static_cast<size_t>(sh.np) * (sh.kp / 32)))) return p->rc;
     if (!(p->d_r = dev_alloc<double>(p, sh.np))) return p->rc;
     if (!(p->d_scratch = dev_alloc<double>(p, static_cast<size_t>(chunks) * sh.np))) return p->rc;
-    if (!(p->d_flag_counts = dev_alloc<unsigned long long>(p, p->mine.size() + 1))) return p->rc;
+    const bool rowsum_in_expand = sh.fused_embed && intacc && !sh.bits_feed;
+    const size_t n_counts = p->mine.size() + 1;
+    p->n_zeroed = n_counts + (rowsum_in_expand ? static_cast<size_t>(sh.np) + (sh.kp / 128 + 2) / 2 : 0);
+    if (!(p->d_flag_counts = dev_alloc<unsigned long long>(p, p->n_zeroed))) return p->rc;
+    if (rowsum_in_expand) {
+      p->d_r_int = reinterpret_cast<long long*>(p->d_flag_counts + n_counts);
+      p->d_ready = reinterpret_cast<uint32_t*>(p->d_r_int + sh.np);
+      if (!(p->h_stamps = pin_alloc<unsigned long long>(p, 2))) return p->rc;
+    }
     if (i8 && !(p->d_flag_u = dev_alloc<double>(p, 1))) return p->rc;
     if (i8 && !(p->d_qerr = dev_alloc<double>(p, sh.kp))) return p->rc;
     if (i8 && !(p->d_qam = dev_alloc<uint32_t>(p, sh.kp))) return p->rc;
-    if (intacc && !(p->d_r_int = dev_alloc<long long>(p, sh.np))) return p->rc;
+    if (intacc && !rowsum_in_expand && !(p->d_r_int = dev_alloc<long long>(p, sh.np))) return p->rc;
     std::string terr;
     if (sh.bits_feed) {
       p->tc = tc_operands_create_bits(p->d_bitsS, sh.np, sh.kp, static_cast<const uint8_t*>(p->d_q0),
@@ -1853,10 +1878,11 @@
   for (auto& p : j->parts) {
     if (!p->embed_timed && p->ev_embed1) {
       cudaSetDevice(p->dc->device);
-      if (cudaEventSynchronize(p->ev_embed1) == cudaSuccess) {
+      if (cudaEventSynchronize(p->d_ready ? p->ev_expand : p->ev_embed1) == cudaSuccess) {
         float a = 0.f, b = 0.f;
         if (cudaEventElapsedTime(&a, p->ev_h2d0, p->ev_h2d1) == cudaSuccess) p->info.h2d_ms = a;
         if (cudaEventElapsedTime(&b, p->ev_embed0, p->ev_embed1) == cudaSuccess) p->info.embed_ms = b;
+        if (p->d_ready) p->info.embed_ms += static_cast<double>(p->h_stamps[1] - p->h_stamps[0]) * 1e-6;
         p->embed_timed = true;
       }
       cudaGetLastError();
diff --git a/frackyfrac_b200/csrc/ptx.cuh b/frackyfrac_b200/csrc/ptx.cuh
--- a/frackyfrac_b200/csrc/ptx.cuh
+++ b/frackyfrac_b200/csrc/ptx.cuh
@@ -245,6 +245,39 @@
          | (static_cast<uint32_t>(m >> 4) << 24);
 }
 
+__device__ __forceinline__ void griddep_launch_dependents() {
+  asm volatile("griddepcontrol.launch_dependents;" ::: "memory");
+}
+__device__ __forceinline__ void griddep_wait() { asm volatile("griddepcontrol.wait;" ::: "memory"); }
+__device__ __forceinline__ void fence_proxy_async_global() {
+  asm volatile("fence.proxy.async.global;" ::: "memory");
+}
+__device__ __forceinline__ void red_release_add(uint32_t* p, uint32_t v) {
+  asm volatile("red.release.gpu.global.add.u32 [%0], %1;" ::"l"(p), "r"(v) : "memory");
+}
+__device__ __forceinline__ uint32_t atom_release_add(uint32_t* p, uint32_t v) {
+  uint32_t old;
+  asm volatile("atom.release.gpu.global.add.u32 %0, [%1], %2;" : "=r"(old) : "l"(p), "r"(v) : "memory");
+  return old;
+}
+__device__ __forceinline__ uint32_t ld_acquire(const uint32_t* p) {
+  uint32_t v;
+  asm volatile("ld.acquire.gpu.global.u32 %0, [%1];" : "=r"(v) : "l"(p) : "memory");
+  return v;
+}
+__device__ __forceinline__ void wait_count(const uint32_t* p, uint32_t target) {
+  uint32_t ns = 32;
+  while (ld_acquire(p) < target) {
+    __nanosleep(ns);
+    if (ns < 256) ns *= 2;
+  }
+}
+__device__ __forceinline__ unsigned long long globaltimer() {
+  unsigned long long t;
+  asm volatile("mov.u64 %0, %%globaltimer;" : "=l"(t));
+  return t;
+}
+
 __device__ __forceinline__ uint32_t cluster_ctarank() {
   uint32_t r;
   asm volatile("mov.u32 %0, %%cluster_ctarank;" : "=r"(r));
diff --git a/frackyfrac_b200/csrc/unweighted_tc.cu b/frackyfrac_b200/csrc/unweighted_tc.cu
--- a/frackyfrac_b200/csrc/unweighted_tc.cu
+++ b/frackyfrac_b200/csrc/unweighted_tc.cu
@@ -104,7 +104,8 @@
                  const long long* __restrict__ r_int, double unit, const Tile* __restrict__ tiles, int32_t n_tiles,
                  int64_t n_samples, int64_t first, float* __restrict__ out, double flag_below,
                  const double* __restrict__ flag_u_ptr, uint32_t* __restrict__ flagged,
-                 unsigned long long* __restrict__ n_flagged, int dbg) {
+                 unsigned long long* __restrict__ n_flagged, int dbg, const uint32_t* __restrict__ ready,
+                 uint32_t ready_target) {
   (void)dbg;
   constexpr bool kI8 = kMode != 0;
   constexpr bool kInt = kMode == 2;
@@ -159,10 +160,16 @@
       const void* mapB = cta == 0 ? static_cast<const void*>(&mapBh) : static_cast<const void*>(&mapBl);
       constexpr int kElems = kI8 ? BKB : BKB / 2;
       TL(long long w_empty = 0;)
+      int kb_ready = ready ? 0 : n_kblocks;
       for (int t = pair; t < n_tiles; t += n_pairs) {
         const Tile tile = tiles[t];
         const int row_a = (tile.tj + static_cast<int>(cta)) * BM, row_b = tile.ti * BN;
         for (int kb = 0; kb < n_kblocks; ++kb) {
+          if (kb >= kb_ready) {
+            ptx::wait_count(ready + kb, ready_target);
+            ptx::fence_proxy_async_global();
+            kb_ready = kb + 1;
+          }
           TL(const long long c0 = clock64();)
           ptx::mbar_wait(empty_bar(stage), phase ^ 1u);
           TL(w_empty += clock64() - c0;)
@@ -287,6 +294,8 @@
         TL(w_tfull += c1 - c0; t_drain += clock64() - c1;)
       }
       TL(const long long c2 = clock64();)
+      if (kInt && ready != nullptr && t == pair)
+        ptx::wait_count(ready + n_kblocks, ready_target * static_cast<uint32_t>(n_kblocks));
       const int64_t j = static_cast<int64_t>(tile.tj + static_cast<int>(cta)) * BM + q * 32 + lane;
       const int64_t i0 = static_cast<int64_t>(tile.ti) * BN + cg * EPI2_COLS;
       static_assert(EPI2_COLS == 32, "r[i] is broadcast from lane n");
@@ -341,6 +350,7 @@
     __syncwarp();
     ptx::tmem_dealloc<2>(tmem_base, TMEM_COLS);
   }
+  ptx::griddep_wait();
 }
 
 namespace bits {
@@ -796,7 +806,8 @@
 
 int launch_unweighted_tc(const TcOperands* ops, const double* r, const Tile* tiles, int32_t n_tiles,
                          int64_t n_samples, int64_t first, float* out, double flag_below,
-                         uint32_t* flagged, unsigned long long* n_flagged, int num_sms, cudaStream_t s) {
+                         uint32_t* flagged, unsigned long long* n_flagged, int num_sms, cudaStream_t s,
+                         const uint32_t* ready, uint32_t ready_target) {
   if (n_tiles <= 0) return 0;
   const int pairs = num_sms / 2;
   const int grid = 2 * (n_tiles < pairs ? n_tiles : pairs);
@@ -809,9 +820,25 @@
   }
 #define FRC_TC2_ARGS ops->mapP, ops->mapBh, ops->mapBl, c.end, c.scale, c.shift, c.n, c.biased ? 1 : 0, r, ops->r_int, \
                      ops->unit, tiles, n_tiles, n_samples, first, out, flag_below, ops->flag_u, flagged, n_flagged, ops->dbg
-  if (ops->i8 && ops->r_int) k_unweighted_tc2<2><<<grid, THREADS2, SMEM2_BYTES, s>>>(FRC_TC2_ARGS);
-  else if (ops->i8) k_unweighted_tc2<1><<<grid, THREADS2, SMEM2_BYTES, s>>>(FRC_TC2_ARGS);
-  else k_unweighted_tc2<0><<<grid, THREADS2, SMEM2_BYTES, s>>>(FRC_TC2_ARGS);
+  if (ready && ops->i8 && ops->r_int) {
+    cudaLaunchAttribute attr[1];
+    attr[0].id = cudaLaunchAttributeProgrammaticStreamSerialization;
+    attr[0].val.programmaticStreamSerializationAllowed = 1;
+    cudaLaunchConfig_t cfg = {};
+    cfg.gridDim = dim3(grid);
+    cfg.blockDim = dim3(THREADS2);
+    cfg.dynamicSmemBytes = SMEM2_BYTES;
+    cfg.stream = s;
+    cfg.attrs = attr;
+    cfg.numAttrs = 1;
+    cudaLaunchKernelEx(&cfg, k_unweighted_tc2<2>, FRC_TC2_ARGS, ready, ready_target);
+  } else if (ops->i8 && ops->r_int) {
+    k_unweighted_tc2<2><<<grid, THREADS2, SMEM2_BYTES, s>>>(FRC_TC2_ARGS, nullptr, 0u);
+  } else if (ops->i8) {
+    k_unweighted_tc2<1><<<grid, THREADS2, SMEM2_BYTES, s>>>(FRC_TC2_ARGS, nullptr, 0u);
+  } else {
+    k_unweighted_tc2<0><<<grid, THREADS2, SMEM2_BYTES, s>>>(FRC_TC2_ARGS, nullptr, 0u);
+  }
 #undef FRC_TC2_ARGS
   return 1;
 }
```

After: 29.60 billion (median of 6 runs). -3.8%, worse.
